# ecker-lab/TreeLearn

Hardware: AMD Instinct MI355X
Metric: Mpoints/sec through sparse U-Net fwd (0.1 m voxel, 40x40 m tile) (higher is better)
Workload: dtype bf16; 1 GPU; config2: single 40x40 m tile, voxel 0.1 m, 1890607 points/tile, 7-level 32-ch sparse U-Net fwd (30.1 M params, random init), 1 tile per GPU; points_per_tile=1890607, tiles_in_flight=4

## Files before the change

### include/treelearn_hip.h

```cpp
#ifndef TREELEARN_HIP_H
#define TREELEARN_HIP_H

#include <stdint.h>

#ifdef __cplusplus
extern "C" {
#endif

typedef void* tl_stream_t;

enum {
  TL_OK = 0,
  TL_ERR_ARG = -1,
  TL_ERR_LAUNCH = -2,
  TL_ERR_UNSUPPORTED = -3
};

enum { TL_F32 = 0, TL_BF16 = 1, TL_F16 = 2 };

int tl_version(void);
int tl_set_tuning(const char* key, int64_t value);
const char* tl_error_string(int code);


// ... 18 lines not shown

int tl_voxel_mean_feats(const float* pf, int C, const int64_t* v2p, int64_t N, int64_t M, int P,
                        int32_t* ws, float* out, tl_stream_t stream);
int tl_voxel_feats(const float* xyz, const float* feats, int F, const int64_t* v2p, int64_t N, int64_t M, int P, int use_coords,
                   int use_feats, int dtype, int32_t* ws, void* out, tl_stream_t stream);


int tl_rulebook_subm(const int32_t* coords, int64_t M, const uint64_t* bitmap, const uint32_t* prefix,
                     const int32_t dims[4], int32_t* nbr, int32_t* compact ,
                     tl_stream_t stream);

int tl_rulebook_down(const int32_t* ccoords, int64_t Mc, const uint64_t* fbitmap, const uint32_t* fprefix,
                     const int32_t fdims[4], int64_t Mf, int32_t* child, int32_t* parent, int32_t* inv, tl_stream_t stream);

int64_t tl_pyramid_ws_words(const int32_t dims0[4], int num_levels, int64_t* level_word_offsets);
int tl_pyramid_build(const int32_t* pcoords, int64_t N, const int32_t dims0[4], const int32_t shape0[3], int num_levels,
                     uint64_t* bitmaps, uint32_t* prefixes, uint32_t* counts, uint32_t* ws, tl_stream_t stream);

typedef struct tl_level {
  int32_t dims[4];
  int64_t n;
  const uint64_t* bitmap;
  const uint32_t* prefix;
  int32_t* coords;
  int32_t* nbr;
  int32_t* compact;
  int32_t* child;
  int32_t* parent;
  int32_t* inv;
  const int32_t* o2n;
  int32_t* inv_packed;
} tl_level;

int tl_rulebooks_build(const tl_level* levels, int num_levels, int32_t* minus_one, int64_t minus_one_words,
                       const int32_t* pcoords, int64_t N, int64_t* v2p, tl_stream_t stream);

#define TL_BLK_HALO_MAX 126
typedef struct tl_blk {
  int32_t* o2n; int32_t* perm; int32_t* coords_new;
  int32_t* unit; int32_t* counter; int32_t* halo; uint32_t* lrb; int32_t* pmask;
  int64_t cap_units;
  int32_t halo_max;
  int32_t reserved;
  int32_t* nn;
} tl_blk;
int64_t tl_blk_ws_words(const int32_t dims[4]);
int tl_blk_build(const uint64_t* bitmap, const uint32_t* prefix, const int32_t dims[4], int64_t n, const tl_blk* out, uint32_t* ws,
                 int phases, tl_stream_t stream);

int tl_rulebook_compact(const int32_t* table, int64_t n, int32_t* compact, tl_stream_t stream);

typedef struct tl_conv_args {
  const void* in;        int64_t in_ld;
  const void* weight;
  const int32_t* table;
  int64_t n_out;         int64_t n_in;
  int32_t K;             int32_t Cin;     int32_t Cout;   int32_t dtype;
  const float* in_scale; const float* in_shift;  int32_t in_relu;  int32_t out_relu;
  const void* residual;  int64_t res_ld;
  const float* out_scale; const float* out_shift;
  void* out;             int64_t out_ld;
  void* out2; int64_t out2_ld; const float* out2_scale; const float* out2_shift; int32_t out2_relu;
  void* out3; int64_t out3_ld; const float* out3_scale; const float* out3_shift; int32_t out3_relu;
  const void* weight_frag;
  int32_t table_one_hot;
  const int32_t* table_compact;
  int32_t in_all_ones;
  int32_t epi_mode;
  double* red_part;
  int32_t* red_nparts;
  const void* bn_x;      int64_t bn_x_ld;
  const float* bn_mean;  const float* bn_rstd;  const float* bn_scale;  const float* bn_shift;  int32_t bn_relu;
  const int32_t* blk_unit; const int32_t* blk_counter; const int32_t* blk_halo; const uint32_t* blk_lrb; const int32_t* blk_pmask;
  const int32_t* table_scatter;
  const void* weight_x3;
} tl_conv_args;

#define TL_EPI_NONE 0
#define TL_EPI_STATS 1
#define TL_EPI_BN_BWD 2
int64_t tl_conv_red_parts(int64_t n_out);

int tl_conv_fwd(const tl_conv_args* args, tl_stream_t stream);

int tl_pack_weight(const float* w_ref, int Cout, int K, int Cin, void* w_packed, int dtype, tl_stream_t stream);
int64_t tl_pack_weight_x3_bytes(int Cout, int K, int Cin);
int tl_pack_weight_x3(const float* w_ref, int Cout, int K, int Cin, void* w_x3, tl_stream_t stream);
int tl_pack_weight_dgrad(const float* w_ref, int Cout, int K, int Cin, int flip, void* w_t, int dtype, tl_stream_t stream);
typedef struct tl_pack_desc {
  const float* src;
  void* dst;
  int32_t Cout, K, Cin, form;
} tl_pack_desc;
int tl_pack_weights_batch(const tl_pack_desc* descs, const int32_t* blocks, int64_t n_blocks, int dtype, tl_stream_t stream);
int tl_pack_weight_frag(const float* w_ref, int Cout, int K, int Cin, void* w_frag, int dtype, tl_stream_t stream);

int64_t tl_conv_wgrad_ws_floats(int64_t n_out, int K, int Cin, int Cout);
int tl_conv_wgrad(const void* x, int64_t x_ld, const void* gout, int64_t g_ld, int dtype, const int32_t* table, int64_t n_out,
                  int64_t n_in, int K, int Cin, int Cout, float* gw, float* ws, tl_stream_t stream);
int tl_conv_wgrad_ref(const void* x, int64_t x_ld, const void* gout, int64_t g_ld, int dtype, const int32_t* table, int64_t n_out,
                      int64_t n_in, int K, int Cin, int Cout, float* gw, float* ws, tl_stream_t stream);

int64_t tl_conv_wgrad_blk_ws_floats(void);
int tl_conv_wgrad_blk(const void* x, int64_t x_ld, const void* gout, int64_t g_ld, int dtype, const int32_t* blk_unit, const int32_t* blk_counter,
                      const int32_t* blk_halo, const uint32_t* blk_lrb, int64_t n, int Cin, int Cout, float* gw, int ref_layout, float* ws,
                      tl_stream_t stream);

int tl_head_mlp(const void* feats, int64_t feats_ld, int dtype, int C, const int64_t* v2p, int64_t N,
                const float* pro_scale, const float* pro_shift,
                const float* w1, const float* b1, const float* w2, const float* b2,
                float* backbone, float* logits, float* offsets, tl_stream_t stream);

int tl_affine_relu(const void* in, int64_t in_ld, void* out, int64_t out_ld, int64_t n, int C, int dtype,
                   const float* scale, const float* shift, int relu, tl_stream_t stream);

int64_t tl_bn_ws_doubles(int64_t n, int C);
int tl_bn_train_stats(const void* x, int64_t ld, int64_t n, int C, int dtype, const float* gamma, const float* beta, float eps,
                      float momentum, double* ws, float* mean, float* rstd, float* scale, float* shift, float* running_mean,
                      float* running_var, int64_t* num_batches_tracked, tl_stream_t stream);
int tl_bn_train_bwd(const void* x, int64_t ld, int x_dtype, const void* dy, int64_t dld, int dy_dtype, int64_t n, int C,
                    const float* mean, const float* rstd, const float* scale, const float* shift, int relu, double* ws,
                    float* dgamma, float* dbeta, void* dx, int64_t xld, const void* dx_add, int64_t dx_add_ld, tl_stream_t stream);

int tl_bn_train_finish(const double* part, int64_t nparts, int64_t n, int C, const float* gamma, const float* beta, float eps, float momentum, float* mean,
                       float* rstd, float* scale, float* shift, float* running_mean, float* running_var, int64_t* num_batches_tracked, tl_stream_t stream);
int tl_bn_train_bwd_from_parts(const void* x, int64_t ld, int x_dtype, const void* g, int64_t gld, int g_dtype, int64_t n, int C, const float* mean,
                               const float* rstd, const float* scale, const float* shift, const double* part, int64_t nparts, float* dgamma, float* dbeta,
                               void* dx, int64_t xld, const void* dx_add, int64_t dx_add_ld, tl_stream_t stream);

int tl_linear_small_f32(const void* x, int64_t x_ld, int dtype, const void* w, int Cin, int Cout, int64_t n, float* out, int64_t out_ld,
                        tl_stream_t stream);

int tl_gather_rows(const void* in, int64_t in_ld, int dtype, int C, int64_t n_rows, const int64_t* idx, int64_t N, void* out, int64_t out_ld, tl_stream_t stream);
int tl_scatter_add_rows(const void* g, int64_t g_ld, int dtype, int C, const int64_t* order, const int64_t* sorted_idx, int64_t N, int64_t n_rows, void* gin,
                        int64_t gin_ld, tl_stream_t stream);

int64_t tl_compact_ws_words(int64_t n);
int tl_compact_rows(const float* in, int C, const uint8_t* mask, int64_t n, float* out, int32_t* count,
                    int32_t* ws, tl_stream_t stream);

typedef struct tl_tile_box {
  float outer[4];
  double inner[4];
  double center[2];
  float half_inner;
} tl_tile_box;
int64_t tl_tile_crop_ws_words(int64_t n);
int tl_tile_crop(const float* xyz, const float* label, const float* feat, int64_t n, int F, const tl_tile_box* box,
                 float* coords, float* out_feat, int64_t* instance_labels, int64_t* semantic_labels,
                 uint8_t* mask_inner, uint8_t* mask_sem, int32_t* count, int32_t* ws, tl_stream_t stream);

int tl_cell_keys(const double* xyz, int64_t n, double cell, double min_bound, const int64_t* base3, int round_input,
                 int64_t* keys, int32_t* err, tl_stream_t stream);
int64_t tl_downsample_ws_words(int64_t n);
int tl_downsample_reduce(const double* xyz, const int64_t* sorted_keys, const int64_t* perm, int64_t n, float* out_xyz,
                         int64_t* first_idx, int64_t* point2vox, int64_t* n_voxels, int32_t* ws, tl_stream_t stream);
int tl_downsample_reduce_r64(const double* xyz, const int64_t* sorted_keys, const int64_t* perm, int64_t n, float* out_xyz,
                             int64_t* first_idx, int64_t* point2vox, int64_t* n_voxels, int32_t* ws, tl_stream_t stream);
int tl_group_mean(const float* src, int64_t n, int C, const int64_t* sorted_keys, const int64_t* perm, double* mean,
                  int64_t* first_idx, int64_t* n_groups, int32_t* ws, tl_stream_t stream);
int tl_verticality(const double* xyz_sorted, const int64_t* sorted_keys, int64_t n, double radius, const int64_t* extent2,
                   float* out, tl_stream_t stream);

int tl_crops_occupancy(const float* xy, int64_t n, const double* x_steps, int x_dim, const double* y_steps, int y_dim, uint8_t* grid,
                       tl_stream_t stream);
int tl_crops_fill(const uint8_t* raw, int x_dim, int y_dim, int how_far_fill, double min_percent_occupied_fill, uint8_t* filled,
// ... 41 lines not shown
                        double* e_w, double* core, void* ws, tl_stream_t stream);
int tl_hdbscan_prim_order_host(const int32_t* e_src, const int32_t* e_dst, const double* e_w, int64_t n, int32_t* o_src,
                               int32_t* o_dst, double* o_w);

int tl_knn_vote(const float* ref_xyz, const int64_t* ref_label, int64_t nr, const float* q_xyz, int64_t nq, int k,
                int64_t* out_label, tl_stream_t stream);
int tl_knn_vote_grid(const float* ref_sorted_xyz, const int64_t* ref_sorted_label, const int64_t* ref_sorted_index, int64_t nr,
                     const int64_t* cell_keys, const int64_t* cell_start, int64_t ncells, const float lo[3], float h, const int32_t dims[3],
                     const float* q_xyz, int64_t nq, int k, int64_t* out_label, tl_stream_t stream);

int tl_eval_contingency(const int64_t* pred, const int64_t* gt, int64_t n, int64_t n_pred, int64_t n_gt, int64_t non_tree_label,
                        int64_t* table, tl_stream_t stream);
enum { TL_EVAL_XY = 0, TL_EVAL_Z = 1 };
int tl_eval_partition(const double* xyz, const int64_t* gt, const int64_t* pred, int64_t n, const int64_t* gt_order, const int64_t* gt_start,
                      int64_t n_gt, const int64_t* pred_order, const int64_t* pred_start, int64_t n_pred, const int64_t* pairs, int64_t m,
                      const double* edges, int n_edges, int mode, int64_t* tp, int64_t* fp, int64_t* fn, double* norm, tl_stream_t stream);

int64_t tl_pointwise_eval_ws_bytes(int64_t n);
int tl_pointwise_eval(const void* logits, const void* offsets, int dtype, const int64_t* semantic_labels, const float* offset_labels,
                      const uint8_t* mask, int64_t n, void* state, void* ws, tl_stream_t stream);

int tl_point_jitter(float* xyz, int64_t n, uint64_t key, tl_stream_t stream);
int64_t tl_train_item_ws_bytes(int64_t n);
int tl_train_item(const float* xyz, const int32_t* instance_label, int64_t n, const double* m, double half_inner, const float* center,
                  int64_t batch_id, int64_t row_offset, float* coords, int64_t* semantic_labels, int64_t* instance_labels,
                  float* offset_labels, uint8_t* masks_inner, uint8_t* masks_off, uint8_t* masks_sem, int64_t* batch_ids, float* centers,
                  void* ws, tl_stream_t stream);

typedef struct {
  double lo[2], h, r, pad, cover_r2, slab_lo, slab_h;
  int32_t nx, ny, nslab, reserved;
} tl_ring_grid;
int tl_ring_lists(const double* ring, int64_t V, const tl_ring_grid* grid, int64_t* cell_cnt, int64_t* slab_cnt, int32_t* cell_seg,
                  int32_t* slab_seg, tl_stream_t stream);
int tl_ring_covered(const double* ring, const tl_ring_grid* grid, const int64_t* cell_start, const int32_t* cell_seg, uint8_t* covered,
                    tl_stream_t stream);
int tl_ring_classify(const void* pts, int dtype_f64, int64_t ld, int64_t n, const double* ring, const tl_ring_grid* grid,
                     const int64_t* slab_start, const int32_t* slab_seg, const int64_t* cell_start, const int32_t* cell_seg,
                     const uint8_t* covered, uint8_t* out, tl_stream_t stream);


#define TL_MAX_LEVELS 8
#define TL_ERR_ARENA (-4)
#define TL_ERR_REACH_ZERO (-5)
#define TL_ERR_BLK (-7)
#define TL_ERR_EXTENT (-6)
typedef struct tl_affine { const float* scale; const float* shift; } tl_affine;
typedef struct tl_weight { const void* w; const void* frag; int32_t K, Cout, Cin, reserved; const void* x3;  } tl_weight;
typedef struct tl_res_desc {
  tl_affine bn0; tl_weight w1; tl_affine bn3; tl_weight w2;
  tl_weight w1x1;
  tl_weight w1_half[2];
} tl_res_desc;
typedef struct tl_ublock_desc {
  int32_t C; int32_t deeper;
  tl_res_desc blocks[2];
  tl_affine bn_down; tl_weight wd;
  tl_affine bn_up; tl_weight wu;
  tl_res_desc tail[2];
  tl_affine bn_cat_l, bn_cat_r;
} tl_ublock_desc;
typedef struct tl_net_desc {
  int32_t dtype;
  int32_t num_levels;
  float voxel_size;
  int32_t has_shape; int32_t spatial_shape[3];
  int32_t blocked;
  int32_t in_channels;
  int32_t use_coords, use_feats;
  int32_t max_points_per_voxel;
  int32_t reserved0;
  tl_weight w_in;
  tl_ublock_desc u[TL_MAX_LEVELS];
  tl_affine out_bn;
  const float* head_w1; const float* head_b1; const float* head_w2; const float* head_b2;
} tl_net_desc;
typedef struct tl_launch_rec {
  int32_t level, kind;
  int32_t K, Cin, Cout, residual, esize, split_part, split_cin, in_prologue;
  int64_t n_out, n_in;
  float ms;
} tl_launch_rec;
typedef struct tl_forward_args {
  const float* xyz; const int64_t* batch_ids; int64_t N; int32_t B; int32_t reserved;
  const float* point_feats;
  void* arena; int64_t arena_bytes;
  float* backbone;
  float* logits; float* offsets;
  tl_stream_t side_stream;
  int64_t needed_bytes;
  int64_t level_n[TL_MAX_LEVELS];
  int32_t blocked_used;
  int32_t launches;
} tl_forward_args;
typedef struct tl_exec tl_exec;
tl_exec* tl_exec_create(void);
void tl_exec_destroy(tl_exec* ex);
int tl_forward(tl_exec* ex, const tl_net_desc* net, tl_forward_args* args, tl_stream_t stream);
int tl_exec_check(tl_exec* ex);
int tl_exec_profile(tl_exec* ex, int enable);
int tl_exec_profile_read(tl_exec* ex, tl_launch_rec* recs, int cap);


#ifdef __cplusplus
}
#endif
#endif
```

### treelearn_amd/_hip.py

```python
import ctypes
import os

import torch

_HERE = os.path.dirname(os.path.abspath(__file__))
LIB_PATH = os.path.join(_HERE, "lib", "libtreelearn_hip.so")

TL_F32, TL_BF16, TL_F16 = 0, 1, 2
TL_OK, TL_ERR_ARG, TL_ERR_UNSUPPORTED = 0, -1, -3
TL_EPI_NONE, TL_EPI_STATS, TL_EPI_BN_BWD = 0, 1, 2
_c = ctypes
_vp, _i64, _i32, _f32 = _c.c_void_p, _c.c_int64, _c.c_int32, _c.c_float


class ConvArgs(_c.Structure):
    _fields_ = [
        ("in_", _vp), ("in_ld", _i64), ("weight", _vp), ("table", _vp),
        ("n_out", _i64), ("n_in", _i64), ("K", _i32), ("Cin", _i32), ("Cout", _i32), ("dtype", _i32),
        ("in_scale", _vp), ("in_shift", _vp), ("in_relu", _i32), ("out_relu", _i32),
        ("residual", _vp), ("res_ld", _i64), ("out_scale", _vp), ("out_shift", _vp),
        ("out", _vp), ("out_ld", _i64),
        ("out2", _vp), ("out2_ld", _i64), ("out2_scale", _vp), ("out2_shift", _vp), ("out2_relu", _i32),
        ("out3", _vp), ("out3_ld", _i64), ("out3_scale", _vp), ("out3_shift", _vp), ("out3_relu", _i32),
        ("weight_frag", _vp), ("table_one_hot", _i32), ("table_compact", _vp),
        ("in_all_ones", _i32), ("epi_mode", _i32), ("red_part", _vp), ("red_nparts", _c.POINTER(_i32)),
        ("bn_x", _vp), ("bn_x_ld", _i64), ("bn_mean", _vp), ("bn_rstd", _vp), ("bn_scale", _vp), ("bn_shift", _vp), ("bn_relu", _i32),
        ("blk_unit", _vp), ("blk_counter", _vp), ("blk_halo", _vp), ("blk_lrb", _vp), ("blk_pmask", _vp), ("table_scatter", _vp),
        ("weight_x3", _vp),
    ]


class TileBox(_c.Structure):
    _fields_ = [("outer", _c.c_float * 4), ("inner", _c.c_double * 4), ("center", _c.c_double * 2), ("half_inner", _c.c_float)]


class Level(_c.Structure):
    _fields_ = [("dims", _c.c_int32 * 4), ("n", _c.c_int64), ("bitmap", _c.c_void_p), ("prefix", _c.c_void_p), ("coords", _c.c_void_p),
                ("nbr", _c.c_void_p), ("compact", _c.c_void_p), ("child", _c.c_void_p), ("parent", _c.c_void_p), ("inv", _c.c_void_p),
                ("o2n", _c.c_void_p), ("inv_packed", _c.c_void_p)]


class Blk(_c.Structure):
    _fields_ = [("o2n", _vp), ("perm", _vp), ("coords_new", _vp), ("unit", _vp), ("counter", _vp), ("halo", _vp), ("lrb", _vp), ("pmask", _vp),
                ("cap_units", _i64), ("halo_max", _i32), ("reserved", _i32), ("nn", _vp)]


class HdbGrid(_c.Structure):
    _fields_ = [("lo", _c.c_double * 2), ("h", _c.c_double), ("levels", _c.c_int32), ("reserved", _c.c_int32)]


TL_MAX_LEVELS = 8
TL_ERR_ARENA, TL_ERR_REACH_ZERO, TL_ERR_EXTENT, TL_ERR_BLK = -4, -5, -6, -7


class Affine(_c.Structure):
    _fields_ = [("scale", _vp), ("shift", _vp)]


class Weight(_c.Structure):
    _fields_ = [("w", _vp), ("frag", _vp), ("K", _i32), ("Cout", _i32), ("Cin", _i32), ("reserved", _i32), ("x3", _vp)]


class ResDesc(_c.Structure):
    _fields_ = [("bn0", Affine), ("w1", Weight), ("bn3", Affine), ("w2", Weight), ("w1x1", Weight), ("w1_half", Weight * 2)]


class UBlockDesc(_c.Structure):
    _fields_ = [("C", _i32), ("deeper", _i32), ("blocks", ResDesc * 2), ("bn_down", Affine), ("wd", Weight), ("bn_up", Affine), ("wu", Weight),
                ("tail", ResDesc * 2), ("bn_cat_l", Affine), ("bn_cat_r", Affine)]


class NetDesc(_c.Structure):
    _fields_ = [("dtype", _i32), ("num_levels", _i32), ("voxel_size", _f32), ("has_shape", _i32), ("spatial_shape", _i32 * 3), ("blocked", _i32),
                ("in_channels", _i32), ("use_coords", _i32), ("use_feats", _i32), ("max_points_per_voxel", _i32), ("reserved0", _i32),
                ("w_in", Weight), ("u", UBlockDesc * TL_MAX_LEVELS), ("out_bn", Affine),
                ("head_w1", _vp), ("head_b1", _vp), ("head_w2", _vp), ("head_b2", _vp)]


class LaunchRec(_c.Structure):
    _fields_ = [("level", _i32), ("kind", _i32), ("K", _i32), ("Cin", _i32), ("Cout", _i32), ("residual", _i32), ("esize", _i32), ("split_part", _i32),
                ("split_cin", _i32), ("in_prologue", _i32), ("n_out", _i64), ("n_in", _i64), ("ms", _f32)]


class ForwardArgs(_c.Structure):
    _fields_ = [("xyz", _vp), ("batch_ids", _vp), ("N", _i64), ("B", _i32), ("reserved", _i32), ("point_feats", _vp), ("arena", _vp), ("arena_bytes", _i64),
                ("backbone", _vp), ("logits", _vp), ("offsets", _vp), ("side_stream", _vp), ("needed_bytes", _i64),
                ("level_n", _i64 * TL_MAX_LEVELS), ("blocked_used", _i32), ("launches", _i32)]


_I4 = _i32 * 4
_I3 = _i32 * 3

PROTOTYPES = {
    "tl_version": (_i32, []),
    "tl_error_string": (_c.c_char_p, [_i32]),
    "tl_set_tuning": (_i32, [_c.c_char_p, _i64]),
    "tl_voxel_point_coords": (_i32, [_vp, _vp, _i64, _i32, _f32, _vp, _vp, _vp, _vp]),
    "tl_voxel_point_coords_one": (_i32, [_vp, _vp, _i64, _f32, _vp, _vp, _vp, _c.POINTER(_i32), _vp]),
    "tl_bitmap_from_points": (_i32, [_vp, _i64, _I4, _vp, _vp]),
    "tl_bitmap_down": (_i32, [_vp, _I4, _I3, _vp, _I4, _vp]),
    "tl_scan_ws_words": (_i64, [_i64]),
    "tl_bitmap_scan": (_i32, [_vp, _i64, _vp, _vp, _vp, _vp]),
    "tl_expand_coords": (_i32, [_vp, _vp, _I4, _vp, _vp]),
    "tl_point_rank": (_i32, [_vp, _i64, _vp, _vp, _I4, _vp, _vp]),
    "tl_voxel_mean_feats": (_i32, [_vp, _i32, _vp, _i64, _i64, _i32, _vp, _vp, _vp]),
    "tl_voxel_feats": (_i32, [_vp, _vp, _i32, _vp, _i64, _i64, _i32, _i32, _i32, _i32, _vp, _vp, _vp]),
    "tl_rulebook_subm": (_i32, [_vp, _i64, _vp, _vp, _I4, _vp, _vp, _vp]),
    "tl_rulebook_down": (_i32, [_vp, _i64, _vp, _vp, _I4, _i64, _vp, _vp, _vp, _vp]),
    "tl_rulebook_compact": (_i32, [_vp, _i64, _vp, _vp]),
    "tl_pyramid_ws_words": (_i64, [_I4, _i32, _c.POINTER(_i64)]),
    "tl_pyramid_build": (_i32, [_vp, _i64, _I4, _I3, _i32, _vp, _vp, _vp, _vp, _vp]),
    "tl_rulebooks_build": (_i32, [_c.POINTER(Level), _i32, _vp, _i64, _vp, _i64, _vp, _vp]),
    "tl_blk_ws_words": (_i64, [_I4]),
    "tl_blk_build": (_i32, [_vp, _vp, _I4, _i64, _c.POINTER(Blk), _vp, _i32, _vp]),
    "tl_conv_fwd": (_i32, [_c.POINTER(ConvArgs), _vp]),
    "tl_conv_red_parts": (_i64, [_i64]),
    "tl_exec_create": (_vp, []),
    "tl_exec_destroy": (None, [_vp]),
    "tl_forward": (_i32, [_vp, _c.POINTER(NetDesc), _c.POINTER(ForwardArgs), _vp]),
    "tl_exec_check": (_i32, [_vp]),
    "tl_exec_profile": (_i32, [_vp, _i32]),
    "tl_exec_profile_read": (_i32, [_vp, _c.POINTER(LaunchRec), _i32]),
    "tl_bn_train_finish": (_i32, [_vp, _i64, _i64, _i32, _vp, _vp, _f32, _f32, _vp, _vp, _vp, _vp, _vp, _vp, _vp, _vp]),
    "tl_bn_train_bwd_from_parts": (_i32, [_vp, _i64, _i32, _vp, _i64, _i32, _i64, _i32, _vp, _vp, _vp, _vp, _vp, _i64, _vp, _vp, _vp, _i64, _vp, _i64, _vp]),
    "tl_pack_weight": (_i32, [_vp, _i32, _i32, _i32, _vp, _i32, _vp]),
    "tl_pack_weight_x3": (_i32, [_vp, _i32, _i32, _i32, _vp, _vp]),
    "tl_pack_weight_x3_bytes": (_i64, [_i32, _i32, _i32]),
    "tl_pack_weight_frag": (_i32, [_vp, _i32, _i32, _i32, _vp, _i32, _vp]),
    "tl_pack_weights_batch": (_i32, [_vp, _vp, _i64, _i32, _vp]),
    "tl_pack_weight_dgrad": (_i32, [_vp, _i32, _i32, _i32, _i32, _vp, _i32, _vp]),
    "tl_conv_wgrad_ws_floats": (_i64, [_i64, _i32, _i32, _i32]),
    "tl_conv_wgrad": (_i32, [_vp, _i64, _vp, _i64, _i32, _vp, _i64, _i64, _i32, _i32, _i32, _vp, _vp, _vp]),
    "tl_conv_wgrad_ref": (_i32, [_vp, _i64, _vp, _i64, _i32, _vp, _i64, _i64, _i32, _i32, _i32, _vp, _vp, _vp]),
    "tl_conv_wgrad_blk_ws_floats": (_i64, []),
    "tl_conv_wgrad_blk": (_i32, [_vp, _i64, _vp, _i64, _i32, _vp, _vp, _vp, _vp, _i64, _i32, _i32, _vp, _i32, _vp, _vp]),
    "tl_head_mlp": (_i32, [_vp, _i64, _i32, _i32, _vp, _i64, _vp, _vp, _vp, _vp, _vp, _vp, _vp, _vp, _vp, _vp]),
    "tl_affine_relu": (_i32, [_vp, _i64, _vp, _i64, _i64, _i32, _i32, _vp, _vp, _i32, _vp]),
    "tl_bn_ws_doubles": (_i64, [_i64, _i32]),
    "tl_bn_train_stats": (_i32, [_vp, _i64, _i64, _i32, _i32, _vp, _vp, _f32, _f32, _vp, _vp, _vp, _vp, _vp, _vp, _vp, _vp, _vp]),
    "tl_bn_train_bwd": (_i32, [_vp, _i64, _i32, _vp, _i64, _i32, _i64, _i32, _vp, _vp, _vp, _vp, _i32, _vp, _vp, _vp, _vp, _i64, _vp, _i64, _vp]),
    "tl_linear_small_f32": (_i32, [_vp, _i64, _i32, _vp, _i32, _i32, _i64, _vp, _i64, _vp]),
    "tl_gather_rows": (_i32, [_vp, _i64, _i32, _i32, _i64, _vp, _i64, _vp, _i64, _vp]),
    "tl_scatter_add_rows": (_i32, [_vp, _i64, _i32, _i32, _vp, _vp, _i64, _i64, _vp, _i64, _vp]),
    "tl_compact_ws_words": (_i64, [_i64]),
    "tl_compact_rows": (_i32, [_vp, _i32, _vp, _i64, _vp, _vp, _vp, _vp]),
    "tl_tile_crop_ws_words": (_i64, [_i64]),
    "tl_tile_crop": (_i32, [_vp, _vp, _vp, _i64, _i32, _vp, _vp, _vp, _vp, _vp, _vp, _vp, _vp, _vp, _vp]),
    "tl_cell_keys": (_i32, [_vp, _i64, _c.c_double, _c.c_double, _vp, _i32, _vp, _vp, _vp]),
    "tl_downsample_ws_words": (_i64, [_i64]),
    "tl_downsample_reduce": (_i32, [_vp, _vp, _vp, _i64, _vp, _vp, _vp, _vp, _vp, _vp]),
    "tl_downsample_reduce_r64": (_i32, [_vp, _vp, _vp, _i64, _vp, _vp, _vp, _vp, _vp, _vp]),
    "tl_group_mean": (_i32, [_vp, _i64, _i32, _vp, _vp, _vp, _vp, _vp, _vp, _vp]),
    "tl_verticality": (_i32, [_vp, _vp, _i64, _c.c_double, _vp, _vp, _vp]),
    "tl_cluster_ws_bytes": (_i64, [_i64]),
    "tl_cluster_grid": (_i32, [_vp, _i64, _c.c_double, _vp, _vp, _vp, _vp]),
    "tl_hdbscan_ws_bytes": (_i64, [_i64]),
    "tl_hdbscan_mst": (_i32, [_vp, _i64, _i32, _vp, _vp, _vp, _vp, _vp, _vp]),
    "tl_hdbscan_labels_host": (_i32, [_vp, _vp, _vp, _i64, _i32, _vp]),
    "tl_hdbscan_prim_order_host": (_i32, [_vp, _vp, _vp, _i64, _vp, _vp, _vp]),
    "tl_hdbscan_grid_plan_ws_bytes": (_i64, []),
    "tl_hdbscan_grid_plan": (_i32, [_vp, _i64, _vp, _vp, _vp]),
    "tl_hdbscan_grid_ws_bytes": (_i64, [_i64, _vp]),
    "tl_hdbscan_grid_ws_bytes_k": (_i64, [_i64, _vp, _i32]),
    "tl_hdbscan_mst_grid": (_i32, [_vp, _i64, _i32, _vp, _vp, _vp, _vp, _vp, _vp, _vp]),
    "tl_knn_vote": (_i32, [_vp, _vp, _i64, _vp, _i64, _i32, _vp, _vp]),
    "tl_knn_vote_grid": (_i32, [_vp, _vp, _vp, _i64, _vp, _vp, _i64, _c.c_float * 3, _f32, _I3, _vp, _i64, _i32, _vp, _vp]),
    "tl_eval_contingency": (_i32, [_vp, _vp, _i64, _i64, _i64, _i64, _vp, _vp]),
    "tl_eval_partition": (_i32, [_vp, _vp, _vp, _i64, _vp, _vp, _i64, _vp, _vp, _i64, _vp, _i64, _vp, _i32, _i32, _vp, _vp, _vp, _vp, _vp]),
    "tl_pointwise_eval_ws_bytes": (_i64, [_i64]),
    "tl_pointwise_eval": (_i32, [_vp, _vp, _i32, _vp, _vp, _vp, _i64, _vp, _vp, _vp]),
    "tl_point_jitter": (_i32, [_vp, _i64, _c.c_uint64, _vp]),
    "tl_train_item_ws_bytes": (_i64, [_i64]),
    "tl_train_item": (_i32, [_vp, _vp, _i64, _c.POINTER(_c.c_double), _c.c_double, _c.POINTER(_f32), _i64, _i64, _vp, _vp, _vp, _vp, _vp, _vp, _vp, _vp, _vp,
                             _vp, _vp]),
    "tl_ring_lists": (_i32, [_vp, _i64, _vp, _vp, _vp, _vp, _vp, _vp]),
    "tl_ring_covered": (_i32, [_vp, _vp, _vp, _vp, _vp, _vp]),
    "tl_crops_occupancy": (_i32, [_vp, _i64, _vp, _i32, _vp, _i32, _vp, _vp]),
    "tl_crops_fill": (_i32, [_vp, _i32, _i32, _i32, _c.c_double, _vp, _vp]),
    "tl_crops_check": (_i32, [_vp, _i32, _vp, _i32, _vp, _vp, _vp, _i64, _c.c_double, _c.c_double, _c.c_double, _vp, _vp, _vp]),
    "tl_crops_ws_words": (_i64, [_i64, _i32]),
    "tl_crops_count": (_i32, [_vp, _i64, _i32, _vp, _vp, _c.c_double, _vp, _vp, _vp]),
    "tl_crops_extract": (_i32, [_vp, _vp, _vp, _i64, _i32, _i32, _vp, _vp, _c.c_double, _vp, _i64, _vp, _vp, _vp, _vp]),
    "tl_outlier_keys": (_i32, [_vp, _i64, _c.c_double * 3, _c.c_double, _I3, _vp, _vp, _vp]),
    "tl_knn_mean_dist": (_i32, [_vp, _vp, _vp, _i64, _c.c_double * 3, _c.c_double, _I3, _i32, _vp, _vp]),
    "tl_sor_ws_doubles": (_i64, [_i64]),
    "tl_sor_keep": (_i32, [_vp, _i64, _c.c_double, _vp, _vp, _vp, _vp]),
    "tl_radius_count": (_i32, [_vp, _vp, _vp, _i64, _c.c_double * 3, _c.c_double, _I3, _c.c_double, _vp, _vp]),
    "tl_ring_classify": (_i32, [_vp, _i32, _i64, _i64, _vp, _vp, _vp, _vp, _vp, _vp, _vp, _vp, _vp]),
}
TL_EVAL_XY, TL_EVAL_Z = 0, 1


class RingGrid(_c.Structure):
    _fields_ = [("lo", _c.c_double * 2), ("h", _c.c_double), ("r", _c.c_double), ("pad", _c.c_double), ("cover_r2", _c.c_double),
                ("slab_lo", _c.c_double), ("slab_h", _c.c_double), ("nx", _i32), ("ny", _i32), ("nslab", _i32), ("reserved", _i32)]

_lib = None

# ... 62 lines not shown
```

### treelearn_amd/csrc/tl_common.h

```cpp
#pragma once
#include <hip/hip_runtime.h>
#include <stdint.h>
#include <atomic>
#include "../../include/treelearn_hip.h"

#define TL_CHECK_LAUNCH()                                   \
  do {                                                      \
    if (hipGetLastError() != hipSuccess) return TL_ERR_LAUNCH; \
  } while (0)

static inline hipStream_t tl_s(tl_stream_t s) { return reinterpret_cast<hipStream_t>(s); }

struct TlAttrOnce {
  std::atomic<uint64_t> done[4];
};
static inline bool tl_lds_attr(TlAttrOnce& once, const void* kernel, int bytes) {
  int dev = 0;
  if (hipGetDevice(&dev) != hipSuccess) return false;
  std::atomic<uint64_t>& w = once.done[(dev >> 6) & 3];
  const uint64_t bit = 1ull << (dev & 63);
  if (w.load(std::memory_order_acquire) & bit) return true;
  if (hipFuncSetAttribute(kernel, hipFuncAttributeMaxDynamicSharedMemorySize, bytes) != hipSuccess) return false;
  w.fetch_or(bit, std::memory_order_release);
  return true;
}

static inline int64_t tl_cdiv(int64_t a, int64_t b) { return (a + b - 1) / b; }

static inline unsigned tl_grid(int64_t work_items, int block) {
  int64_t g = tl_cdiv(work_items, block);
  if (g < 1) g = 1;
  if (g > 256 * 16) g = 256 * 16;
  return (unsigned)g;
}

struct TlDims {
  int B, X, Y, Z, Zw;
};
static inline TlDims tl_dims(const int32_t d[4]) {
  TlDims r{d[0], d[1], d[2], d[3], (d[3] + 63) >> 6};
  return r;
}
__host__ __device__ static inline int64_t tl_nwords(const TlDims& d) { return (int64_t)d.B * d.X * d.Y * d.Zw; }

__device__ __forceinline__ int64_t tl_col_word(const TlDims& d, int b, int x, int y) {
  return (((int64_t)b * d.X + x) * d.Y + y) * d.Zw;
}

__device__ __forceinline__ int tl_rank_at(const uint64_t* __restrict__ bm, const uint32_t* __restrict__ pf,
                                          int64_t wc, int z) {
  const int64_t w = wc + (z >> 6);
  const uint64_t word = bm[w];
  const uint64_t bit = 1ull << (z & 63);
  if (!(word & bit)) return -1;
  return (int)(pf[w] + __popcll(word & (bit - 1)));
}

bool tl_conv_one_hot_direct_enabled(int64_t n_out);
```

### treelearn_amd/csrc/tl_conv.hip

```cpp
#include "tl_conv_internal.h"
#include <atomic>
#include <string.h>

namespace {

template <typename T>
__global__ void __launch_bounds__(256) k_conv_generic(ConvP p) {
  const T* in = (const T*)p.in; const T* w = (const T*)p.w; const T* res = (const T*)p.res;
  const int64_t total = p.n_out * p.Cout;
  for (int64_t t = (int64_t)blockIdx.x * blockDim.x + threadIdx.x; t < total; t += (int64_t)gridDim.x * blockDim.x) {
    const int64_t o = t / p.Cout; const int j = (int)(t % p.Cout);
    float acc = 0.f;
    for (int k = 0; k < p.K; ++k) {
      const int64_t idx = p.table ? (int64_t)p.table[(int64_t)k * p.n_out + o] : o;
      if (idx < 0) continue;
      const T* x = in + idx * p.in_ld;
      const T* wr = w + ((int64_t)k * p.Cout + j) * p.Cin;
      for (int c = 0; c < p.Cin; ++c) {
        float v = ld_elem(x + c);
        if (p.in_scale) v = fmaf(v, p.in_scale[c], p.in_shift[c]);
        if (p.in_relu) v = fmaxf(v, 0.f);
        if (sizeof(T) == 2) v = __bfloat162float(__float2bfloat16(v));
        acc = fmaf(v, ld_elem(wr + c), acc);
      }
// ... 237 lines not shown
    else reinterpret_cast<__hip_bfloat16*>(d.dst)[t] = __float2bfloat16(v);
  }
}

template <typename T>
__global__ void k_affine_relu(const T* __restrict__ in, int64_t in_ld, T* __restrict__ out, int64_t out_ld, int64_t n, int C,
                              const float* __restrict__ scale, const float* __restrict__ shift, int relu) {
  const int64_t total = n * C;
  for (int64_t t = (int64_t)blockIdx.x * blockDim.x + threadIdx.x; t < total; t += (int64_t)gridDim.x * blockDim.x) {
    const int64_t r = t / C; const int c = (int)(t % C);
    float v = ld_elem(in + r * in_ld + c);
    if (scale) v = fmaf(v, scale[c], shift[c]);
    if (relu) v = fmaxf(v, 0.f);
    st_elem(out + r * out_ld + c, v);
  }
}

template <int T16>
__global__ void __launch_bounds__(256) k_affine_relu_v8(const void* __restrict__ in, int64_t in_ld, void* __restrict__ out, int64_t out_ld, int64_t n, int C,
                                                        const float* __restrict__ scale, const float* __restrict__ shift, int relu) {
  const int vpr = C >> 3;
  const int64_t total = n * vpr, stride = (int64_t)gridDim.x * 256;
  int64_t v = (int64_t)blockIdx.x * 256 + threadIdx.x;
  if (v >= total) return;
  const int c0 = (int)(v % vpr) * 8;
  float sc[8], sh[8];
#pragma unroll
  for (int q = 0; q < 8; ++q) { sc[q] = scale ? scale[c0 + q] : 1.f; sh[q] = scale ? shift[c0 + q] : 0.f; }
  for (; v < total; v += stride) {
    const int64_t r = v / vpr;
    float x[8];
    typedef _Float16 hx2 __attribute__((ext_vector_type(2)));
    if constexpr (T16 == 1) {
      const u32x4 q4 = __builtin_nontemporal_load(reinterpret_cast<const u32x4*>((const uint16_t*)in + r * in_ld + c0));
#pragma unroll
      for (int q = 0; q < 4; ++q) { x[2 * q] = bf16_lo(q4[q]); x[2 * q + 1] = bf16_hi(q4[q]); }
    } else if constexpr (T16 == 2) {
      const u32x4 q4 = *reinterpret_cast<const u32x4*>((const uint16_t*)in + r * in_ld + c0);
      const uint32_t w0 = q4[0], w1 = q4[1], w2 = q4[2], w3 = q4[3];
      const uint32_t ws[4] = {w0, w1, w2, w3};
#pragma unroll
      for (int q = 0; q < 4; ++q) { const hx2 h = __builtin_bit_cast(hx2, ws[q]); x[2 * q] = (float)h[0]; x[2 * q + 1] = (float)h[1]; }
    } else {
      const f32x4* s4 = reinterpret_cast<const f32x4*>((const float*)in + r * in_ld + c0);
      const f32x4 a = __builtin_nontemporal_load(s4), b = __builtin_nontemporal_load(s4 + 1);
#pragma unroll
      for (int q = 0; q < 4; ++q) { x[q] = a[q]; x[q + 4] = b[q]; }
    }
#pragma unroll
    for (int q = 0; q < 8; ++q) { x[q] = fmaf(x[q], sc[q], sh[q]); if (relu) x[q] = fmaxf(x[q], 0.f); }
    if constexpr (T16 == 1) {
      u32x4 o;
#pragma unroll
      for (int q = 0; q < 4; ++q) o[q] = pack_bf16x2(x[2 * q], x[2 * q + 1]);
      *reinterpret_cast<u32x4*>((uint16_t*)out + r * out_ld + c0) = o;
    } else if constexpr (T16 == 2) {
      u32x4 o;
#pragma unroll
      for (int q = 0; q < 4; ++q) { const hx2 h = {(_Float16)x[2 * q], (_Float16)x[2 * q + 1]}; o[q] = __builtin_bit_cast(uint32_t, h); }
      *reinterpret_cast<u32x4*>((uint16_t*)out + r * out_ld + c0) = o;
    } else {
      f32x4* d = reinterpret_cast<f32x4*>((float*)out + r * out_ld + c0);
      d[0] = f32x4{x[0], x[1], x[2], x[3]}; d[1] = f32x4{x[4], x[5], x[6], x[7]};
    }
  }
}

}

static int64_t g_small_rows = kSmallRows;
extern int g_small_mode;
extern int g_wgrad_dense;
extern int64_t g_wgrad_dense_min_rows;
extern int g_wgrad_rows;
extern int g_wgrad_dma;
static int g_stream = 1;
static int g_streamq = 1;
static int g_streamq_x3 = 1;
static int g_direct = 1;
static int g_direct_oh = 1;
static int g_blk = 1;
static int g_up = 1;

bool tl_conv_one_hot_direct_enabled(int64_t n_out) { return g_direct && g_direct_oh && n_out > g_small_rows; }

extern "C" {

int tl_set_tuning(const char* key, int64_t value) {
  if (!key) return TL_ERR_ARG;
  if (!strcmp(key, "direct")) { g_direct = (int)value; return TL_OK; }
  if (!strcmp(key, "blk")) { g_blk = (int)value; return TL_OK; }
  if (!strcmp(key, "up")) { g_up = (int)value; return TL_OK; }
  if (!strcmp(key, "direct_oh")) { g_direct_oh = (int)value; return TL_OK; }
  if (!strcmp(key, "stream")) { g_stream = (int)value; return TL_OK; }
  if (!strcmp(key, "streamq")) { g_streamq = (int)value; return TL_OK; }
  if (!strcmp(key, "streamq_x3")) { if (value != 0 && value != 1) return TL_ERR_ARG; g_streamq_x3 = (int)value; return TL_OK; }
  if (!strcmp(key, "small_rows")) { g_small_rows = value; return TL_OK; }
  if (!strcmp(key, "small_mode")) { g_small_mode = (int)value; return TL_OK; }
  if (!strcmp(key, "wgrad_dense")) { g_wgrad_dense = (int)value; return TL_OK; }
  if (!strcmp(key, "wgrad_rows")) { g_wgrad_rows = (int)value; return TL_OK; }
  if (!strcmp(key, "wgrad_dma")) { g_wgrad_dma = (int)value; return TL_OK; }
  if (!strcmp(key, "wgrad_dense_min_rows")) { g_wgrad_dense_min_rows = value; return TL_OK; }
  return TL_ERR_ARG;
}

int tl_conv_fwd(const tl_conv_args* a, tl_stream_t stream) {
  if (!a || !a->in || !a->weight || !a->out || a->n_out <= 0 || a->K <= 0 || a->K > 27 || a->Cin <= 0 || a->Cout <= 0) return TL_ERR_ARG;
  const bool has_blk = a->blk_unit && a->blk_counter && a->blk_halo && a->blk_lrb && a->K == 27;
  if (!a->table && a->K != 1 && !has_blk && !(a->in_all_ones && a->blk_pmask)) return TL_ERR_ARG;
  if ((a->in_scale == nullptr) != (a->in_shift == nullptr)) return TL_ERR_ARG;
  if ((a->out_scale == nullptr) != (a->out_shift == nullptr)) return TL_ERR_ARG;
  if (a->dtype != TL_F32 && a->dtype != TL_BF16 && a->dtype != TL_F16) return TL_ERR_ARG;
  const bool f16 = a->dtype == TL_F16;
  const int dt = f16 ? TL_BF16 : a->dtype;
  const auto L_direct = f16 ? tl_launch_conv_direct_f16 : tl_launch_conv_direct;
  const auto L_ones27 = f16 ? tl_launch_conv_ones27_f16 : tl_launch_conv_ones27;
  const auto L_stream = f16 ? tl_launch_conv_stream_f16 : tl_launch_conv_stream;
  const auto L_streamq = f16 ? tl_launch_conv_streamq_f16 : tl_launch_conv_streamq;
  const auto L_small = f16 ? tl_launch_conv_small_f16 : tl_launch_conv_small;
  const auto L_tinycin = f16 ? tl_launch_conv_tinycin_f16 : tl_launch_conv_tinycin;
  const auto L_blk = f16 ? tl_launch_conv_blk_f16 : tl_launch_conv_blk;
  const auto L_up = f16 ? tl_launch_conv_up_f16 : tl_launch_conv_up;
  ConvP p;
  p.in = a->in; p.in_ld = a->in_ld; p.w = a->weight; p.w_frag = a->weight_frag;
  p.w_x3 = (a->dtype == TL_F32 && a->Cin % 32 == 0 && ((uintptr_t)a->weight_x3) % 16 == 0) ? a->weight_x3 : nullptr; p.table = a->table; p.ctab = (a->K == 27) ? a->table_compact : nullptr; p.n_out = a->n_out; p.n_in = a->n_in;
  p.K = a->K; p.Cin = a->Cin; p.Cout = a->Cout; p.in_scale = a->in_scale; p.in_shift = a->in_shift;
  p.in_relu = a->in_relu; p.out_relu = a->out_relu; p.res = a->residual; p.res_ld = a->res_ld;
  p.out_scale = a->out_scale; p.out_shift = a->out_shift; p.out = a->out; p.out_ld = a->out_ld;
  p.out2 = a->out2; p.out2_ld = a->out2_ld; p.out2_scale = a->out2_scale; p.out2_shift = a->out2_shift; p.out2_relu = a->out2_relu;
  p.out3 = a->out3; p.out3_ld = a->out3_ld; p.out3_scale = a->out3_scale; p.out3_shift = a->out3_shift; p.out3_relu = a->out3_relu;
  if ((a->out2_scale == nullptr) != (a->out2_shift == nullptr) || (a->out3_scale == nullptr) != (a->out3_shift == nullptr)) return TL_ERR_ARG;
  p.nblk = (int)tl_cdiv(a->n_out, TM);
  p.one_hot = a->table != nullptr ? a->table_one_hot : 0;
  p.blk_unit = has_blk ? a->blk_unit : nullptr; p.blk_counter = a->blk_counter; p.blk_halo = a->blk_halo; p.blk_lrb = a->blk_lrb;
  p.blk_pmask = a->K == 27 ? a->blk_pmask : nullptr;
  p.epi_mode = a->epi_mode; p.red_part = a->red_part; p.red_nparts = a->red_nparts; p.bn_x = a->bn_x; p.bn_x_ld = a->bn_x_ld;
  p.bn_mean = a->bn_mean; p.bn_rstd = a->bn_rstd; p.bn_scale = a->bn_scale; p.bn_shift = a->bn_shift; p.bn_relu = a->bn_relu;
  const bool train = a->epi_mode != TL_EPI_NONE;
  if (train) {
    if ((a->epi_mode != TL_EPI_STATS && a->epi_mode != TL_EPI_BN_BWD) || !a->red_part || ((uintptr_t)a->red_part) % 8) return TL_ERR_ARG;
    if (a->epi_mode == TL_EPI_BN_BWD) {
      if (!a->bn_x || !a->bn_mean || !a->bn_rstd || !a->bn_scale || !a->bn_shift) return TL_ERR_ARG;
      if (a->bn_x_ld % 8 || ((uintptr_t)a->bn_x) % 16 || ((uintptr_t)a->bn_mean) % 16 || ((uintptr_t)a->bn_rstd) % 16 || ((uintptr_t)a->bn_scale) % 16 ||
          ((uintptr_t)a->bn_shift) % 16)
        return TL_ERR_UNSUPPORTED;
    }
    if (a->red_nparts) *a->red_nparts = 0;
  }
  hipStream_t s = tl_s(stream);
  if (p.one_hot == 2) {
    const bool shape = a->K == 8 && a->Cin == 64 && a->Cout == 32 && !train && !a->in_scale && !a->in_relu && g_direct && g_direct_oh;
    if (!shape || !(dt == TL_BF16 || (dt == TL_F32 && p.w_x3))) return TL_ERR_UNSUPPORTED;
    return L_direct(p, dt, s);
  }
  const bool vec_ok = (a->in_ld % 8 == 0) && (((uintptr_t)a->in) % 16 == 0) && (((uintptr_t)a->weight) % 16 == 0);
  const bool out_vec = (a->out_ld % 8 == 0) && (((uintptr_t)a->out) % 16 == 0) &&
                       (!a->out2 || (a->out2_ld % 8 == 0 && ((uintptr_t)a->out2) % 16 == 0)) && (!a->out3 || (a->out3_ld % 8 == 0 && ((uintptr_t)a->out3) % 16 == 0));
  if (a->in_all_ones && !train && (dt == TL_BF16 || (dt == TL_F32 && !f16)) && out_vec && (g_direct || !a->table) && ((uintptr_t)a->weight) % 4 == 0 && !a->residual) {
    const int rc = L_ones27(p, dt, s);
    if (rc != TL_ERR_UNSUPPORTED) return rc;
  }
  if (has_blk && dt == TL_BF16 && g_blk && vec_ok && out_vec && (!a->residual || (a->res_ld % 8 == 0 && ((uintptr_t)a->residual) % 16 == 0)) &&
      (!a->out_scale || (((uintptr_t)a->out_scale) % 4 == 0 && ((uintptr_t)a->out_shift) % 4 == 0)) && (!a->in_relu || a->in_scale)) {
    const int rc = L_blk(p, s);
    if (rc != TL_ERR_UNSUPPORTED) return rc;
  }
  if (has_blk && a->dtype == TL_F32 && p.w_x3 && g_blk && !train) {
    const int rc = tl_launch_conv_blk_x3(p, s);
    if (rc != TL_ERR_UNSUPPORTED) return rc;
  }
  if (!a->table && a->K != 1) return TL_ERR_UNSUPPORTED;
  if (a->table_scatter && p.one_hot && g_up && !train && dt == TL_BF16 && vec_ok && out_vec &&
      (!a->out_scale || (((uintptr_t)a->out_scale) % 16 == 0 && ((uintptr_t)a->out_shift) % 16 == 0))) {
    const int rc = L_up(p, a->table_scatter, s);
    if (rc != TL_ERR_UNSUPPORTED) return rc;
  }
  if (dt == TL_BF16 && a->Cin == 4 && a->Cout == 32 && g_direct && out_vec && ((uintptr_t)a->in) % 8 == 0 && ((uintptr_t)a->weight) % 16 == 0 &&
      (!a->residual || (a->res_ld % 8 == 0 && ((uintptr_t)a->residual) % 16 == 0))) {
    const int rc = L_direct(p, TL_BF16, s);
    if (rc != TL_ERR_UNSUPPORTED) return rc;
  }
  if (!train && a->Cin <= 8 && a->Cout % 8 == 0 && a->Cout <= 64 && !a->in_scale && !a->in_relu && out_vec) return L_tinycin(p, dt, s);
  if (!train && vec_ok && a->n_out <= g_small_rows && a->Cin % 32 == 0 && a->Cout % 32 == 0) return L_small(p, dt, s);
  if (train && a->n_out <= g_small_rows) return TL_ERR_UNSUPPORTED;
  const bool aligned = (a->in_ld % 4 == 0) && (((uintptr_t)a->in) % 16 == 0) && (((uintptr_t)a->weight) % 16 == 0) &&
                       (!a->in_scale || (((uintptr_t)a->in_scale) % 16 == 0 && ((uintptr_t)a->in_shift) % 16 == 0));
  if (p.w_x3 && a->Cin >= 256) {
    if (dt == TL_F32 && !train && g_stream && aligned && out_vec && a->Cin % 64 == 0 && a->Cout % 32 == 0 && !a->in_scale && !a->in_relu && !a->residual &&
        !a->out2 && !a->out3 && a->n_out > g_small_rows && (!a->out_scale || (((uintptr_t)a->out_scale) % 16 == 0 && ((uintptr_t)a->out_shift) % 16 == 0))) {
      ConvP p1 = p;
      p1.Cin = a->Cin / 2; p1.out_scale = nullptr; p1.out_shift = nullptr; p1.out_relu = 0;
      const int rc1 = L_stream(p1, TL_F32, s);
      if (rc1 == TL_OK) {
        ConvP p2 = p;
        p2.Cin = a->Cin / 2; p2.in = static_cast<const float*>(a->in) + a->Cin / 2;
        p2.w_x3 = static_cast<const char*>(p.w_x3) + (size_t)a->K * a->Cout * (a->Cin / 2) * 4;
        p2.res = a->out; p2.res_ld = a->out_ld;
        return L_stream(p2, TL_F32, s);
      }
      if (rc1 != TL_ERR_UNSUPPORTED) return rc1;
    }
    p.w_x3 = nullptr;
  }
  if (dt == TL_F32 && aligned && out_vec && a->Cin % 32 == 0 && a->Cout % 32 == 0 && !a->in_scale && !a->in_relu &&
      (!a->residual || (a->res_ld % 4 == 0 && ((uintptr_t)a->residual) % 16 == 0)) &&
      (!a->out_scale || (((uintptr_t)a->out_scale) % 16 == 0 && ((uintptr_t)a->out_shift) % 16 == 0))) {
    if (g_direct) { const int rc = L_direct(p, TL_F32, s); if (rc != TL_ERR_UNSUPPORTED) return rc; }
    if (g_stream && g_streamq && g_streamq_x3 && p.w_x3 && !train && a->n_out > g_small_rows) {
      const int rc = tl_launch_conv_streamq_x3(p, s);
      if (rc != TL_ERR_UNSUPPORTED) return rc;
    }
    if (g_stream) { const int rc = L_stream(p, TL_F32, s); if (rc != TL_ERR_UNSUPPORTED) return rc; }
  }
  if (train && dt == TL_F32) return TL_ERR_UNSUPPORTED;
  if (dt == TL_F32 && !f16 && vec_ok && a->n_out <= 4 * g_small_rows && a->Cin % 32 == 0 && a->Cout % 32 == 0 && !a->in_scale && !a->in_relu)
    return L_small(p, dt, s);
  if (dt == TL_F32 && aligned && a->Cin % KC == 0 && a->Cout % 32 == 0 && a->Cout <= 224) {
    switch (a->Cout / 32) {
      case 1: return launch_mfma_f32<1>(p, s);
      case 2: return launch_mfma_f32<2>(p, s);
      case 3: return launch_mfma_f32<3>(p, s);
      case 4: return launch_mfma_f32<4>(p, s);
      case 5: return launch_mfma_f32<5>(p, s);
      case 6: return launch_mfma_f32<6>(p, s);
      case 7: return launch_mfma_f32<7>(p, s);
    }
  }
  if (dt == TL_BF16 && aligned && vec_ok && out_vec && a->Cin % 32 == 0 && a->Cout % 32 == 0 && a->Cout <= 224 &&
      (!a->residual || (a->res_ld % 8 == 0 && ((uintptr_t)a->residual) % 16 == 0)) &&
      (!a->out_scale || (((uintptr_t)a->out_scale) % 16 == 0 && ((uintptr_t)a->out_shift) % 16 == 0)))
  {
    if (p.one_hot && g_direct && g_direct_oh && a->K == 8 && a->Cin == 64 && a->Cout == 32) {
      const int rc = L_direct(p, TL_BF16, s);
      if (rc != TL_ERR_UNSUPPORTED) return rc;
    }
    if (p.one_hot && g_stream && a->K == 8) {
      const int rc = L_stream(p, TL_BF16, s);
      if (rc != TL_ERR_UNSUPPORTED) return rc;
    }
    if (g_direct) {
      const int rc = L_direct(p, TL_BF16, s);
      if (rc != TL_ERR_UNSUPPORTED) return rc;
    }
    if (g_stream && g_streamq) {
      const int rc = L_streamq(p, s);
      if (rc != TL_ERR_UNSUPPORTED) return rc;
    }
    if (g_stream) {
      const int rc = L_stream(p, TL_BF16, s);
      if (rc != TL_ERR_UNSUPPORTED) return rc;
    }
    if (train) return TL_ERR_UNSUPPORTED;
    return f16 ? tl_launch_conv_bf16_f16(p, s) : tl_launch_conv_bf16(p, s);
  }
  if (train || f16) return TL_ERR_UNSUPPORTED;
  {
    const int rc = tl_launch_conv_tinycout(p, dt, s);
    if (rc != TL_ERR_UNSUPPORTED) return rc;
  }
  const unsigned g = tl_grid(a->n_out * a->Cout, 256);
  if (dt == TL_F32) k_conv_generic<float><<<g, 256, 0, s>>>(p);
  else k_conv_generic<__hip_bfloat16><<<g, 256, 0, s>>>(p);
  TL_CHECK_LAUNCH();
  return TL_OK;
}

int64_t tl_conv_red_parts(int64_t n_out) {
  const int64_t a = tl_cdiv(n_out > 0 ? n_out : 1, 256);
  return a > 2048 ? a : 2048;
}

int tl_pack_weight(const float* w_ref, int Cout, int K, int Cin, void* w_packed, int dtype, tl_stream_t stream) {
  if (!w_ref || !w_packed || Cout <= 0 || K <= 0 || Cin <= 0 || (dtype != TL_F32 && dtype != TL_BF16 && dtype != TL_F16)) return TL_ERR_ARG;
  k_pack_weight<<<tl_grid((int64_t)Cout * K * Cin, 256), 256, 0, tl_s(stream)>>>(w_ref, Cout, K, Cin, w_packed, dtype);
  TL_CHECK_LAUNCH();
  return TL_OK;
}

int64_t tl_pack_weight_x3_bytes(int Cout, int K, int Cin) {
  if (Cout <= 0 || K <= 0 || Cin <= 0 || Cin % 32) return -1;
  const int64_t one = (int64_t)K * Cout * Cin * 4;
  return (Cin < 256 && Cout % 32 == 0) ? 2 * one : one;
}

int tl_pack_weight_x3(const float* w_ref, int Cout, int K, int Cin, void* w_x3, tl_stream_t stream) {
  if (!w_ref || !w_x3 || Cout <= 0 || K <= 0 || Cin <= 0 || Cin % 32) return TL_ERR_ARG;
  k_pack_weight_x3<<<tl_grid((int64_t)Cout * K * Cin * 2, 256), 256, 0, tl_s(stream)>>>(w_ref, Cout, K, Cin, reinterpret_cast<uint16_t*>(w_x3));
  TL_CHECK_LAUNCH();
  return TL_OK;
}

int tl_pack_weight_dgrad(const float* w_ref, int Cout, int K, int Cin, int flip, void* w_t, int dtype, tl_stream_t stream) {
  if (!w_ref || !w_t || Cout <= 0 || K <= 0 || Cin <= 0 || (dtype != TL_F32 && dtype != TL_BF16 && dtype != TL_F16)) return TL_ERR_ARG;
  k_pack_weight_dgrad<<<tl_grid((int64_t)Cout * K * Cin, 256), 256, 0, tl_s(stream)>>>(w_ref, Cout, K, Cin, flip, w_t, dtype);
  TL_CHECK_LAUNCH();
  return TL_OK;
}

int tl_pack_weights_batch(const tl_pack_desc* descs, const int32_t* blocks, int64_t n_blocks, int dtype, tl_stream_t stream) {
  if (!descs || !blocks || n_blocks <= 0 || n_blocks > 0x7FFFFFFF || (dtype != TL_F32 && dtype != TL_BF16 && dtype != TL_F16)) return TL_ERR_ARG;
  k_pack_batch<<<(unsigned)n_blocks, 256, 0, tl_s(stream)>>>(descs, reinterpret_cast<const int2*>(blocks), dtype);
  TL_CHECK_LAUNCH();
  return TL_OK;
}

int tl_pack_weight_frag(const float* w_ref, int Cout, int K, int Cin, void* w_frag, int dtype, tl_stream_t stream) {
  if (!w_ref || !w_frag || Cout <= 0 || K <= 0 || Cin <= 0 || Cout % 32 || Cin % 32 || (dtype != TL_F32 && dtype != TL_BF16 && dtype != TL_F16)) return TL_ERR_ARG;
  k_pack_weight_frag<<<tl_grid((int64_t)Cout * K * Cin / 8, 256), 256, 0, tl_s(stream)>>>(w_ref, Cout, K, Cin, w_frag, dtype);
  TL_CHECK_LAUNCH();
  return TL_OK;
}

int tl_affine_relu(const void* in, int64_t in_ld, void* out, int64_t out_ld, int64_t n, int C, int dtype, const float* scale,
                   const float* shift, int relu, tl_stream_t stream) {
  if (!in || !out || n <= 0 || C <= 0 || (scale == nullptr) != (shift == nullptr)) return TL_ERR_ARG;
  if ((dtype == TL_F32 || dtype == TL_BF16 || dtype == TL_F16) && C % 8 == 0 && in_ld % 8 == 0 && out_ld % 8 == 0 && ((uintptr_t)in) % 16 == 0 && ((uintptr_t)out) % 16 == 0) {
    const int vpr = C / 8;
    int64_t gv = tl_cdiv(n * vpr, 256 * 4);
    if (gv > 256 * 16) gv = 256 * 16;
    gv = tl_cdiv(gv * 256, (int64_t)vpr * 256) * vpr;
    if (dtype == TL_BF16) k_affine_relu_v8<1><<<(unsigned)gv, 256, 0, tl_s(stream)>>>(in, in_ld, out, out_ld, n, C, scale, shift, relu);
    else if (dtype == TL_F16) k_affine_relu_v8<2><<<(unsigned)gv, 256, 0, tl_s(stream)>>>(in, in_ld, out, out_ld, n, C, scale, shift, relu);
    else k_affine_relu_v8<0><<<(unsigned)gv, 256, 0, tl_s(stream)>>>(in, in_ld, out, out_ld, n, C, scale, shift, relu);
    TL_CHECK_LAUNCH();
    return TL_OK;
  }
  const unsigned g = tl_grid(n * C, 256);
  if (dtype == TL_F32) k_affine_relu<float><<<g, 256, 0, tl_s(stream)>>>((const float*)in, in_ld, (float*)out, out_ld, n, C, scale, shift, relu);
  else if (dtype == TL_BF16) k_affine_relu<__hip_bfloat16><<<g, 256, 0, tl_s(stream)>>>((const __hip_bfloat16*)in, in_ld, (__hip_bfloat16*)out, out_ld, n, C, scale, shift, relu);
  else if (dtype == TL_F16) k_affine_relu<_Float16><<<g, 256, 0, tl_s(stream)>>>((const _Float16*)in, in_ld, (_Float16*)out, out_ld, n, C, scale, shift, relu);
  else return TL_ERR_ARG;
  TL_CHECK_LAUNCH();
  return TL_OK;
}

}
```

### treelearn_amd/csrc/tl_conv_direct.hip

```cpp
#include "tl_conv_internal.h"
#include <atomic>

namespace {


template <bool BF16, int K, int NB, int UN, int G, int WAVES, bool CT = false, bool TR = false, bool OH = false, bool X3 = false>
__global__ void __launch_bounds__(WAVES * 64) k_conv_direct(ConvP p, int ntiles, int walk) {
  static_assert(!X3 || (!BF16 && !TR), "the split-bf16 contraction: fp32 rows, inference");
  constexpr int EB = BF16 ? 2 : 4;
  constexpr int UB = 32 * EB;
  constexpr int NJ = UB / 32;
  constexpr int SLOTS = UB / 16;
  constexpr int COUT = NB * 32;
  constexpr int NG = (K + G - 1) / G;
  constexpr int EP = COUT + 4;
  extern __shared__ __attribute__((aligned(16))) char smem[];
  char* Ws = smem;
  float* Es = reinterpret_cast<float*>(smem + (size_t)K * UN * COUT * UB);
  double* Ds = reinterpret_cast<double*>(smem + (size_t)K * UN * COUT * UB + (size_t)WAVES * 32 * EP * 4);

  const int tid = threadIdx.x, lane = tid & 63, wv = tid >> 6;
  const int fi = lane & 31, fh = lane >> 5;
  auto swz_of = [](int n) { return BF16 ? ((n >> 2) & 3) : ((n >> 1) & 7); };

// ... 332 lines not shown
      acc = h16_mfma(af, bfrag[s], acc);
    }
#pragma unroll
    for (int r = 0; r < 16; ++r) ew[((r & 3) + 8 * (r >> 2) + 4 * fh) * EP + fi] = acc[r];
    __builtin_amdgcn_fence(__ATOMIC_RELEASE, "wavefront");
    __builtin_amdgcn_wave_barrier();
    if constexpr (TR) {
      float r0 = 0.f, r1 = 0.f;
      epi_block32<true, EP>(p, ew, lane, (int64_t)tile * 32, 0, r0, r1);
      if (lane < 32) { Ds[wv][0][lane] += (double)r0; Ds[wv][1][lane] += (double)r1; }
    } else {
#pragma unroll
      for (int e0 = 0; e0 < 2; ++e0) {
        const int e = lane + e0 * 64, rr = e >> 2, cvv = e & 3;
        const int64_t orow = (int64_t)tile * 32 + rr;
        if (orow < p.n_out) {
          const f32x4 v0 = *reinterpret_cast<const f32x4*>(ew + rr * EP + cvv * 8), v1 = *reinterpret_cast<const f32x4*>(ew + rr * EP + cvv * 8 + 4);
          float v[8] = {v0[0], v0[1], v0[2], v0[3], v1[0], v1[1], v1[2], v1[3]};
          epi_views8<true>(p, orow, cvv * 8, v);
        }
      }
    }
    __builtin_amdgcn_fence(__ATOMIC_RELEASE, "wavefront");
    __builtin_amdgcn_wave_barrier();
  }
  if constexpr (TR) {
    __syncthreads();
    for (int e = threadIdx.x; e < 64; e += WAVES * 64) {
      double t = 0.0;
      for (int w = 0; w < WAVES; ++w) t += Ds[w][e >> 5][e & 31];
      p.red_part[(int64_t)blockIdx.x * 64 + e] = t;
    }
  }
}

template <bool BF16>
__global__ void __launch_bounds__(256) k_conv_ones27(ConvP p) {
  __shared__ __attribute__((aligned(16))) float S[27][32];
  for (int e = threadIdx.x; e < 27 * 32; e += 256) {
    float t = 0.f;
    if constexpr (BF16) {
      const uint16_t* w = (const uint16_t*)p.w;
      for (int c = 0; c < p.Cin; ++c) t += bf16_lo((uint32_t)w[(int64_t)e * p.Cin + c]);
    } else {
      const float* w = (const float*)p.w;
      for (int c = 0; c < p.Cin; ++c) t += w[(int64_t)e * p.Cin + c];
    }
    S[e >> 5][e & 31] = t;
  }
  __syncthreads();
  const int32_t* mask = p.blk_pmask ? p.blk_pmask : p.ctab + (int64_t)9 * p.n_out;
  const int64_t total = p.n_out * 4;
  for (int64_t t = (int64_t)blockIdx.x * 256 + threadIdx.x; t < total; t += (int64_t)gridDim.x * 256) {
    const int64_t row = t >> 2; const int c0 = (int)(t & 3) * 8;
    uint32_t m = (uint32_t)mask[row];
    float v[8] = {0.f, 0.f, 0.f, 0.f, 0.f, 0.f, 0.f, 0.f};
    while (m) {
      const int k = __builtin_ctz(m); m &= m - 1;
      const f32x4 a = *reinterpret_cast<const f32x4*>(&S[k][c0]), b = *reinterpret_cast<const f32x4*>(&S[k][c0 + 4]);
#pragma unroll
      for (int q = 0; q < 4; ++q) { v[q] += a[q]; v[q + 4] += b[q]; }
    }
    epi_views8<BF16>(p, row, c0, v);
  }
}

template <bool BF16, int K, int NB, int UN, int G, int WAVES, bool CT = false, bool TR = false, bool OH = false, bool X3 = false>
int launch(const ConvP& p_, hipStream_t s) {
  ConvP p = p_;
  if constexpr (X3) {
    if (p.epi_mode != TL_EPI_NONE) return TL_ERR_UNSUPPORTED;
    p.w = p.w_x3;
  }
  if constexpr (!TR && BF16) {
    if (p.epi_mode != TL_EPI_NONE) return launch<BF16, K, NB, UN, G, WAVES, CT, true, OH>(p, s);
  } else if constexpr (!TR) {
    if (p.epi_mode != TL_EPI_NONE) return TL_ERR_UNSUPPORTED;
  }
  if constexpr (TR && NB >= 3) return TL_ERR_UNSUPPORTED;
  else {
  constexpr int UB = BF16 ? 64 : 128;
  const size_t lds = (size_t)K * UN * NB * 32 * UB + (size_t)WAVES * 32 * (NB * 32 + 4) * 4 + (TR ? (size_t)WAVES * 2 * NB * 32 * 8 : 0);
  if (lds > 160 * 1024) return TL_ERR_UNSUPPORTED;
  static TlAttrOnce attr_once;
  if (!tl_lds_attr(attr_once, reinterpret_cast<const void*>(&k_conv_direct<BF16, K, NB, UN, G, WAVES, CT, TR, OH, X3>), 160 * 1024)) return TL_ERR_LAUNCH;
  const int ntiles = (int)tl_cdiv(p.n_out, 32);
  const int per_cu = (int)((160 * 1024) / lds) < 1 ? 1 : (int)((160 * 1024) / lds);
  int grid = 256 * (per_cu > 2 ? 2 : per_cu);
  const int need = (int)tl_cdiv(ntiles, WAVES);
  if (grid > need) grid = need;
  k_conv_direct<BF16, K, NB, UN, G, WAVES, CT, TR, OH, X3><<<grid, WAVES * 64, lds, s>>>(p, ntiles, 0);
  if (p.red_nparts) *p.red_nparts = grid;
  return hipGetLastError() == hipSuccess ? TL_OK : TL_ERR_LAUNCH;
  }
}

template <bool BF16, int K, int G>
int dispatch(const ConvP& p, hipStream_t s) {
  const int nb = p.Cout / 32, un = p.Cin / 32;
  const size_t wbytes = (size_t)K * p.Cout * p.Cin * (BF16 ? 2 : 4);
  if constexpr (BF16 && K == 27) {
    if (p.ctab && nb == 1 && un == 1) return launch<true, 27, 1, 1, G, 16, true>(p, s);
    if (p.ctab && nb == 1 && un == 2) return launch<true, 27, 1, 2, G, 8, true>(p, s);
  }
  if constexpr (BF16 && K == 8) {
    if (p.one_hot && nb == 1 && un == 2) return launch<true, 8, 1, 2, G, 16, false, false, true>(p, s);
  }
  if constexpr (BF16 && K == 1) {
    if (nb == 2 && un == 4) return launch<true, 1, 2, 4, 1, 16>(p, s);
    if (nb == 3 && un == 6) return launch<true, 1, 3, 6, 1, 8>(p, s);
    if (nb == 4 && un == 8) return launch<true, 1, 4, 8, 1, 8>(p, s);
  }
  if constexpr (!BF16 && K == 1) {
    if (nb == 2 && un == 4 && p.epi_mode == TL_EPI_NONE) {
      if (p.w_x3) return launch<false, 1, 2, 4, 1, 8, false, false, false, true>(p, s);
      return launch<false, 1, 2, 4, 1, 8>(p, s);
    }
  }
  if constexpr (!BF16 && K == 8) {
    if (p.one_hot && p.w_x3 && p.epi_mode == TL_EPI_NONE && nb == 1 && un == 2) return launch<false, 8, 1, 2, G, 12, false, false, true, true>(p, s);
  }
#define TL_D(NB_, UN_)                                                                                               \
  if (nb == NB_ && un == UN_) {                                                                                      \
    if constexpr (BF16) return wbytes <= 64 * 1024 ? launch<true, K, NB_, UN_, G, 16>(p, s) : launch<true, K, NB_, UN_, G, 8>(p, s); \
    else {                                                                                                           \
      if (p.w_x3 && p.epi_mode == TL_EPI_NONE)        \
        return launch<false, K, NB_, UN_, (G > 2 ? 2 : G), (K == 27 && NB_ == 1 && UN_ == 1 ? 11 : 8), false, false, false, true>(p, s);         \
      return launch<false, K, NB_, UN_, (G > 2 ? 2 : G), 8>(p, s);                                                   \
    }                                                                                                                \
  }
  TL_D(1, 1) TL_D(1, 2) TL_D(2, 1) TL_D(2, 2) TL_D(2, 3) TL_D(3, 2) TL_D(1, 3) TL_D(3, 1)
#undef TL_D
  return TL_ERR_UNSUPPORTED;
}

}

int tl_launch_conv_ones27(const ConvP& p, int dtype, hipStream_t s) {
  if (p.K != 27 || p.Cout != 32 || (!p.ctab && !p.blk_pmask) || p.Cin <= 0 || p.Cin > 64 || p.in_scale || p.in_relu || p.epi_mode != TL_EPI_NONE) return TL_ERR_UNSUPPORTED;
  if (dtype == TL_BF16) k_conv_ones27<true><<<tl_grid(p.n_out * 4, 256), 256, 0, s>>>(p);
  else k_conv_ones27<false><<<tl_grid(p.n_out * 4, 256), 256, 0, s>>>(p);
  return hipGetLastError() == hipSuccess ? TL_OK : TL_ERR_LAUNCH;
}


int tl_launch_conv_direct(const ConvP& p, int dtype, hipStream_t s) {
  if (p.in_scale || p.in_relu) return TL_ERR_UNSUPPORTED;
  if (p.one_hot == 2 && !(p.K == 8 && p.Cin == 64 && p.Cout == 32 && p.epi_mode == TL_EPI_NONE && (dtype == TL_BF16 || p.w_x3))) return TL_ERR_UNSUPPORTED;
  const int eb = dtype == TL_BF16 ? 2 : 4;
  if (dtype == TL_BF16 && p.Cin == 4 && p.Cout == 32 && p.K <= 28 && p.table && p.in_ld % 4 == 0 && (int64_t)p.n_in * p.in_ld * 2 < 0xFFFF0000ll) {
    const int ntiles = (int)tl_cdiv(p.n_out, 32);
    int grid = (int)tl_cdiv(ntiles, 8);
    if (grid > 2048) grid = 2048;
    if (p.epi_mode != TL_EPI_NONE) {
      if (p.ctab && p.K == 27) k_conv_in4<8, true, true><<<grid, 512, 0, s>>>(p, ntiles);
      else k_conv_in4<8, false, true><<<grid, 512, 0, s>>>(p, ntiles);
    } else if (p.ctab && p.K == 27) k_conv_in4<8, true><<<grid, 512, 0, s>>>(p, ntiles);
    else k_conv_in4<8><<<grid, 512, 0, s>>>(p, ntiles);
    if (p.red_nparts) *p.red_nparts = grid;
    return hipGetLastError() == hipSuccess ? TL_OK : TL_ERR_LAUNCH;
  }
  if (p.Cin % 32 || p.Cout % 32) return TL_ERR_UNSUPPORTED;
  const int64_t ld_b = p.in_ld * eb, in_bytes = (p.n_in - 1) * ld_b + (int64_t)p.Cin * eb;
  if (!(in_bytes > 0 && in_bytes + 2 * ld_b < 0xFFFFFFFFll)) return TL_ERR_UNSUPPORTED;
  if ((size_t)p.K * p.Cout * p.Cin * eb > 112 * 1024) return TL_ERR_UNSUPPORTED;
  if (dtype == TL_BF16) {
    switch (p.K) {
      case 27: return dispatch<true, 27, 3>(p, s);
      case 8: return dispatch<true, 8, 2>(p, s);
      case 1: return dispatch<true, 1, 1>(p, s);
    }
  } else {
    switch (p.K) {
      case 27: return dispatch<false, 27, 3>(p, s);
      case 8: return dispatch<false, 8, 2>(p, s);
      case 1: return dispatch<false, 1, 1>(p, s);
    }
  }
  return TL_ERR_UNSUPPORTED;
}
```

### treelearn_amd/csrc/tl_conv_internal.h

```cpp
#pragma once
#include "tl_common.h"
#include <hip/hip_bf16.h>
#include "tl_half.h"

#ifdef TL_F16_BUILD
#define tl_launch_conv_direct tl_launch_conv_direct_f16
#define tl_launch_conv_ones27 tl_launch_conv_ones27_f16
#define tl_launch_conv_stream tl_launch_conv_stream_f16
#define tl_launch_conv_streamq tl_launch_conv_streamq_f16
#define tl_launch_conv_small tl_launch_conv_small_f16
#define tl_launch_conv_tinycin tl_launch_conv_tinycin_f16
#define tl_launch_conv_bf16 tl_launch_conv_bf16_f16
#define tl_launch_conv_blk tl_launch_conv_blk_f16
#define tl_launch_conv_up tl_launch_conv_up_f16
#define g_small_mode g_small_mode_f16
#endif

typedef float f32x16 __attribute__((ext_vector_type(16)));
typedef float f32x4 __attribute__((ext_vector_type(4)));
typedef uint32_t u32x4 __attribute__((ext_vector_type(4)));
typedef short s16x8 __attribute__((ext_vector_type(8)));

struct ConvP {
  const void* in; int64_t in_ld;
  const void* w;
  const void* w_frag;
  const void* w_x3;
  const int32_t* table;
  const int32_t* ctab;
  int64_t n_out, n_in;
  int K, Cin, Cout;
  const float* in_scale; const float* in_shift; int in_relu, out_relu;
  const void* res; int64_t res_ld;
  const float* out_scale; const float* out_shift;
  void* out; int64_t out_ld;
  void* out2; int64_t out2_ld; const float* out2_scale; const float* out2_shift; int out2_relu;
  void* out3; int64_t out3_ld; const float* out3_scale; const float* out3_shift; int out3_relu;
  int nblk;
  int epi_mode;
  double* red_part;
  int32_t* red_nparts;
  const void* bn_x; int64_t bn_x_ld;
  const float* bn_mean; const float* bn_rstd; const float* bn_scale; const float* bn_shift; int bn_relu;
  int one_hot;
  const int32_t* blk_unit; const int32_t* blk_counter; const int32_t* blk_halo; const uint32_t* blk_lrb; const int32_t* blk_pmask;
};

static __device__ __forceinline__ float ld_elem(const float* p) { return *p; }
static __device__ __forceinline__ float ld_elem(const __hip_bfloat16* p) { return h16_lo((uint32_t)*reinterpret_cast<const uint16_t*>(p)); }
static __device__ __forceinline__ void st_elem(float* p, float v) { *p = v; }
static __device__ __forceinline__ float ld_elem(const _Float16* p) { return (float)*p; }
static __device__ __forceinline__ void st_elem(_Float16* p, float v) { *p = (_Float16)v; }
static __device__ __forceinline__ void st_elem(__hip_bfloat16* p, float v) { *reinterpret_cast<uint16_t*>(p) = (uint16_t)(h16_pack2(v, 0.f) & 0xFFFFu); }

static __device__ __forceinline__ int xcd_tile(int b, int n) {
  const int q = n >> 3, r = n & 7, x = b & 7, i = b >> 3;
  return (x < r ? x * (q + 1) : r * (q + 1) + (x - r) * q) + i;
}


typedef __bf16 bf16x8 __attribute__((ext_vector_type(8)));

static __device__ __forceinline__ uint32_t pack_bf16x2(float lo, float hi) { return h16_pack2(lo, hi); }
static __device__ __forceinline__ float bf16_lo(uint32_t u) { return h16_lo(u); }
static __device__ __forceinline__ float bf16_hi(uint32_t u) { return h16_hi(u); }

template <bool BF16>
static __device__ __forceinline__ void epi_store1(void* base, int64_t ld, const float* sc, const float* sh, int relu, int64_t row, int j, float y) {
  if (sc) y = fmaf(y, sc[j], sh[j]);
  if (relu) y = fmaxf(y, 0.f);
  if constexpr (BF16) ((uint16_t*)base)[row * ld + j] = (uint16_t)(pack_bf16x2(y, 0.f) & 0xFFFFu);
  else ((float*)base)[row * ld + j] = y;
}
template <bool BF16>
static __device__ __forceinline__ void epi_store8(void* base, int64_t ld, const float* sc, const float* sh, int relu, int64_t row, int c0, const float (&y)[8]) {
  float v[8];
#pragma unroll
  for (int q = 0; q < 8; ++q) v[q] = y[q];
  if (sc) {
    const f32x4 a0 = *reinterpret_cast<const f32x4*>(sc + c0), a1 = *reinterpret_cast<const f32x4*>(sc + c0 + 4);
    const f32x4 b0 = *reinterpret_cast<const f32x4*>(sh + c0), b1 = *reinterpret_cast<const f32x4*>(sh + c0 + 4);
#pragma unroll
    for (int q = 0; q < 4; ++q) { v[q] = fmaf(v[q], a0[q], b0[q]); v[q + 4] = fmaf(v[q + 4], a1[q], b1[q]); }
  }
  if (relu) {
#pragma unroll
    for (int q = 0; q < 8; ++q) v[q] = fmaxf(v[q], 0.f);
  }
  if constexpr (BF16) {
    u32x4 o;
#pragma unroll
    for (int q = 0; q < 4; ++q) o[q] = pack_bf16x2(v[2 * q], v[2 * q + 1]);
    *reinterpret_cast<u32x4*>((uint16_t*)base + row * ld + c0) = o;
  } else {
    f32x4* d = reinterpret_cast<f32x4*>((float*)base + row * ld + c0);
    d[0] = f32x4{v[0], v[1], v[2], v[3]}; d[1] = f32x4{v[4], v[5], v[6], v[7]};
  }
}

template <bool BF16>
static __device__ __forceinline__ void mma16(f32x16& acc, const u32x4& a, const u32x4& b) {
  if constexpr (BF16) {
    acc = h16_mfma(a, b, acc);
  } else {
    const f32x4 af = __builtin_bit_cast(f32x4, a), bf = __builtin_bit_cast(f32x4, b);
    acc = __builtin_amdgcn_mfma_f32_32x32x2f32(af[0], bf[0], acc, 0, 0, 0);
    acc = __builtin_amdgcn_mfma_f32_32x32x2f32(af[1], bf[1], acc, 0, 0, 0);
    acc = __builtin_amdgcn_mfma_f32_32x32x2f32(af[2], bf[2], acc, 0, 0, 0);
    acc = __builtin_amdgcn_mfma_f32_32x32x2f32(af[3], bf[3], acc, 0, 0, 0);
  }
}
static __device__ __forceinline__ uint32_t x3_pack2(float a, float b) {
  typedef __bf16 v2 __attribute__((ext_vector_type(2)));
  const v2 v = {(__bf16)a, (__bf16)b};
  return __builtin_bit_cast(uint32_t, v);
}
static __device__ __forceinline__ void x3_split8(const u32x4& a0, const u32x4& a1, u32x4& hi, u32x4& lo) {
#pragma unroll
  for (int q = 0; q < 2; ++q) {
    const uint32_t u0 = a0[2 * q], u1 = a0[2 * q + 1], v0 = a1[2 * q], v1 = a1[2 * q + 1];
    hi[q] = __builtin_amdgcn_perm(u1, u0, 0x07060302u);
    hi[2 + q] = __builtin_amdgcn_perm(v1, v0, 0x07060302u);
    lo[q] = x3_pack2(__uint_as_float(u0) - __uint_as_float(u0 & 0xFFFF0000u), __uint_as_float(u1) - __uint_as_float(u1 & 0xFFFF0000u));
    lo[2 + q] = x3_pack2(__uint_as_float(v0) - __uint_as_float(v0 & 0xFFFF0000u), __uint_as_float(v1) - __uint_as_float(v1 & 0xFFFF0000u));
  }
}
static __device__ __forceinline__ void mma16_x3(f32x16& acc, const u32x4& ah, const u32x4& al, const u32x4& bh, const u32x4& bl) {
  acc = __builtin_amdgcn_mfma_f32_32x32x16_bf16(__builtin_bit_cast(bf16x8, al), __builtin_bit_cast(bf16x8, bh), acc, 0, 0, 0);
  acc = __builtin_amdgcn_mfma_f32_32x32x16_bf16(__builtin_bit_cast(bf16x8, ah), __builtin_bit_cast(bf16x8, bl), acc, 0, 0, 0);
// ... 198 lines not shown
```

### treelearn_amd/csrc/tl_conv_stream.hip

```cpp
#include "tl_conv_internal.h"
#include <atomic>

namespace {

constexpr int WAVES = 8;
constexpr int NT = WAVES * 64;

template <bool BF16, int K, int NB, int UN, int DA, int RB, int OCC, bool OH = false, bool X3 = false>
__global__ void __launch_bounds__(NT, OCC) k_conv_stream(ConvP p) {
  static_assert(!X3 || !BF16, "the split-bf16 contraction reads fp32 rows");
  constexpr int EB = BF16 ? 2 : 4, UB = 32 * EB, NJ = UB / 32, SLOTS = UB / 16;
  constexpr int COUT = NB * 32, CIN = UN * 32;
  constexpr int BROW = CIN * EB + 16;
  constexpr int BSLOTS = UN * SLOTS;
  constexpr int BVEC = COUT * BSLOTS;
  constexpr int BPT = (BVEC + NT - 1) / NT;
  constexpr int EP = 32 + 4;
  constexpr int WROWS = 32 * RB;
  extern __shared__ __attribute__((aligned(16))) char smem[];
  char* Bs = smem;
  float* Es = reinterpret_cast<float*>(smem);

  const int tid = threadIdx.x, lane = tid & 63, wv = tid >> 6;
  const int fi = lane & 31, fh = lane >> 5;
// ... 97 lines not shown
#pragma unroll
        for (int J = 0; J < 2; ++J) {
          u32x4 ah[RB], al[RB];
          if constexpr (OH) {
#pragma unroll
            for (int rb = 0; rb < RB; ++rb) {
              if (k == 0) x3_split8(a1[rb][c][2 * J], a1[rb][c][2 * J + 1], ah1[rb][c][J], al1[rb][c][J]);
              const bool mine = idx[k][rb] >= 0;
#pragma unroll
              for (int q = 0; q < 4; ++q) { ah[rb][q] = mine ? ah1[rb][c][J][q] : 0u; al[rb][q] = mine ? al1[rb][c][J][q] : 0u; }
            }
          } else {
#pragma unroll
            for (int rb = 0; rb < RB; ++rb) x3_split8(a[k % DA][rb][c][2 * J], a[k % DA][rb][c][2 * J + 1], ah[rb], al[rb]);
          }
          u32x4 bh[NB], blo[NB];
#pragma unroll
          for (int nb = 0; nb < NB; ++nb) {
            const char* bp = bl + nb * 32 * BROW + (c * SLOTS + 2 * J + fh) * 16;
            bh[nb] = *reinterpret_cast<const u32x4*>(bp); blo[nb] = *reinterpret_cast<const u32x4*>(bp + 64);
          }
#pragma unroll
          for (int rb = 0; rb < RB; ++rb) {
#pragma unroll
            for (int nb = 0; nb < NB; ++nb) acc[rb][nb] = __builtin_amdgcn_mfma_f32_32x32x16_bf16(__builtin_bit_cast(bf16x8, al[rb]), __builtin_bit_cast(bf16x8, bh[nb]), acc[rb][nb], 0, 0, 0);
#pragma unroll
            for (int nb = 0; nb < NB; ++nb) acc[rb][nb] = __builtin_amdgcn_mfma_f32_32x32x16_bf16(__builtin_bit_cast(bf16x8, ah[rb]), __builtin_bit_cast(bf16x8, blo[nb]), acc[rb][nb], 0, 0, 0);
#pragma unroll
            for (int nb = 0; nb < NB; ++nb) acc[rb][nb] = __builtin_amdgcn_mfma_f32_32x32x16_bf16(__builtin_bit_cast(bf16x8, ah[rb]), __builtin_bit_cast(bf16x8, bh[nb]), acc[rb][nb], 0, 0, 0);
          }
        }
    } else
#pragma unroll
    for (int c = 0; c < UN; ++c)
#pragma unroll
      for (int j = 0; j < NJ; ++j) {
#pragma unroll
        for (int nb = 0; nb < NB; ++nb) {
          const int slot = c * SLOTS + 2 * j + fh;
          const u32x4 bf = *reinterpret_cast<const u32x4*>(bl + nb * 32 * BROW + slot * 16);
#pragma unroll
          for (int rb = 0; rb < RB; ++rb) {
            if constexpr (OH) {
              const u32x4 z = {0u, 0u, 0u, 0u};
              mma16<BF16>(acc[rb][nb], idx[k][rb] >= 0 ? a1[rb][c][j] : z, bf);
            } else mma16<BF16>(acc[rb][nb], a[k % DA][rb][c][j], bf);
          }
        }
      }
    if constexpr (!OH) { if (k + DA < K) issue_a(k + DA, a[k % DA]); }
    if (k + 1 < K) __syncthreads();
  }

  __syncthreads();
  float* ew = Es + wv * 32 * EP;
  float red0[NB], red1[NB];
#pragma unroll
  for (int nb = 0; nb < NB; ++nb) { red0[nb] = 0.f; red1[nb] = 0.f; }
#pragma unroll
  for (int rb = 0; rb < RB; ++rb)
#pragma unroll
    for (int nb = 0; nb < NB; ++nb) {
#pragma unroll
      for (int r = 0; r < 16; ++r) ew[((r & 3) + 8 * (r >> 2) + 4 * fh) * EP + fi] = acc[rb][nb][r];
      __builtin_amdgcn_fence(__ATOMIC_RELEASE, "wavefront");
      __builtin_amdgcn_wave_barrier();
      epi_block32<BF16, EP>(p, ew, lane, r0 + rb * 32, nb * 32, red0[nb], red1[nb]);
      __builtin_amdgcn_fence(__ATOMIC_RELEASE, "wavefront");
      __builtin_amdgcn_wave_barrier();
    }
  if (p.epi_mode != TL_EPI_NONE) epi_finish_wg<WAVES, EP, NB>(p, Es, tid, red0, red1);
}

template <bool BF16, int K, int NB, int UN, int DA, int RB, bool OH = false, bool X3 = false>
int launch(ConvP p, hipStream_t s) {
  if constexpr (X3) p.w = p.w_x3;
  constexpr int EB = BF16 ? 2 : 4;
  constexpr int BPTL = (NB * 32 * UN * (BF16 ? 4 : 8) + NT - 1) / NT;
  constexpr int VG = RB * NB * 16 + DA * RB * UN * (BF16 ? 8 : 16) + (K <= 8 ? 8 : 27) * RB + 4 * BPTL * (DA > 2 ? DA - 1 : 1) + 20;
  constexpr int OCC = (OH && X3) ? 2 : ((VG <= 120 || (X3 && NB * UN <= 4)) ? 4 : 2);
  const size_t wt = 2 * (size_t)NB * 32 * (UN * 32 * EB + 16), ep = (size_t)WAVES * 32 * 36 * 4;
  const size_t lds = wt > ep ? wt : ep;
  if (lds > 160 * 1024) return TL_ERR_UNSUPPORTED;
  static TlAttrOnce attr_once;
  if (!tl_lds_attr(attr_once, reinterpret_cast<const void*>(&k_conv_stream<BF16, K, NB, UN, DA, RB, OCC, OH, X3>), 160 * 1024)) return TL_ERR_LAUNCH;
  p.nblk = (int)tl_cdiv(p.n_out, WAVES * 32 * RB);
  k_conv_stream<BF16, K, NB, UN, DA, RB, OCC, OH, X3><<<p.nblk, NT, lds, s>>>(p);
  if (p.red_nparts) *p.red_nparts = p.nblk;
  return hipGetLastError() == hipSuccess ? TL_OK : TL_ERR_LAUNCH;
}

template <bool BF16, int K>
int dispatch(const ConvP& p, hipStream_t s) {
  const int nb = p.Cout / 32, un = p.Cin / 32;
  if constexpr (BF16 && K == 8) {
    if (p.one_hot) {
      if (nb == 2 && un == 3) return launch<true, 8, 2, 3, 1, 1, true>(p, s);
      if (nb == 1 && un == 2) return launch<true, 8, 1, 2, 1, 1, true>(p, s);
      if (nb == 3 && un == 4) return launch<true, 8, 3, 4, 1, 1, true>(p, s);
    }
  }
  if constexpr (!BF16 && K == 8) {
    if (p.one_hot == 1 && p.w_x3 && p.epi_mode == TL_EPI_NONE) {
      if (nb == 2 && un == 3) return launch<false, 8, 2, 3, 1, 1, true, true>(p, s);
      if (nb == 3 && un == 4) return launch<false, 8, 3, 4, 1, 1, true, true>(p, s);
    }
  }
  if constexpr (BF16 && K == 8) {
    if (!p.one_hot && nb == 2 && un == 1) return launch<true, 8, 2, 1, 3, 2>(p, s);
  }
#define TL_S(NB_, UN_, DB_, RB_, DF_)                                                                \
  if (nb == NB_ && un == UN_) {                                                                      \
    if constexpr (BF16) return launch<true, K, NB_, UN_, DB_, RB_>(p, s);                            \
    else {                                                                                           \
      if (p.w_x3) return launch<false, K, NB_, UN_, 1, 1, false, true>(p, s);    \
      return launch<false, K, NB_, UN_, DF_, 1>(p, s);                                               \
    }                                                                                                \
  }
  TL_S(2, 2, 3, 1, 2) TL_S(2, 4, 2, 1, 1) TL_S(3, 3, 1, 2, 1) TL_S(3, 6, 1, 1, 1) TL_S(4, 4, 2, 1, 1) TL_S(2, 3, 3, 1, 1) TL_S(3, 2, 3, 1, 2)
  TL_S(3, 4, 2, 1, 1) TL_S(4, 3, 2, 1, 1) TL_S(1, 2, 3, 1, 2) TL_S(2, 1, 3, 1, 2) TL_S(1, 1, 3, 1, 2)
#undef TL_S
  return TL_ERR_UNSUPPORTED;
}

}

int tl_launch_conv_stream(const ConvP& p, int dtype, hipStream_t s) {
  if (p.in_scale || p.in_relu) return TL_ERR_UNSUPPORTED;
  const int eb = dtype == TL_BF16 ? 2 : 4;
  const int64_t ld_b = p.in_ld * eb, in_bytes = (p.n_in - 1) * ld_b + (int64_t)p.Cin * eb;
  if (!(in_bytes > 0 && in_bytes + 2 * ld_b < 0xFFFFFFFFll)) return TL_ERR_UNSUPPORTED;
  if (dtype == TL_BF16) {
    switch (p.K) {
      case 27: return dispatch<true, 27>(p, s);
      case 8: return dispatch<true, 8>(p, s);
    }
  } else {
    switch (p.K) {
      case 27: return dispatch<false, 27>(p, s);
      case 8: return dispatch<false, 8>(p, s);
    }
  }
  return TL_ERR_UNSUPPORTED;
}
```

### treelearn_amd/csrc/tl_conv_streamq.hip

```cpp
#include "tl_conv_internal.h"
#include <atomic>
#include <type_traits>

namespace {

template <int CTRL>
static __device__ __forceinline__ uint32_t qperm(uint32_t v) {
  return (uint32_t)__builtin_amdgcn_mov_dpp((int)v, CTRL, 0xf, 0xf, true);
}

static __device__ __forceinline__ void quad_transpose(const u32x4 (&S)[4], u32x4 (&F)[4], bool o0, bool o1) {
  u32x4 T[4];
#pragma unroll
  for (int i1 = 0; i1 < 2; ++i1)
#pragma unroll
    for (int d = 0; d < 4; ++d) {
      const uint32_t P = S[2 * i1][d], Q = S[2 * i1 + 1][d];
      const uint32_t Pn = qperm<0xB1>(P), Qn = qperm<0xB1>(Q);
      T[2 * i1][d] = o0 ? Qn : P;
      T[2 * i1 + 1][d] = o0 ? Q : Pn;
    }
#pragma unroll
  for (int x0 = 0; x0 < 2; ++x0)
#pragma unroll
// ... 152 lines not shown
    for (int pp = 0; pp < PN; ++pp)
#pragma unroll
      for (int s = 0; s < 4; ++s)
#pragma unroll
        for (int nb = 0; nb < NB; ++nb) {
          const u32x4 bf = *reinterpret_cast<const u32x4*>(bl + nb * 32 * BROW + (pp * 8 + s) * 16);
#pragma unroll
          for (int rb = 0; rb < RB; ++rb) {
            mma16<true>(acc[rb][nb], F[rb][pp][s], bf);
          }
        }
    if (k + DA < KV) { issue_a(k + DA, a[U % DA]); if (k + DA + 1 < KV) read_idx(k + DA + 1); }
    if (k + 1 < KV) __syncthreads();
  };
  if constexpr (X3 && !UL) {
    for (int k0 = 0; k0 < KV; k0 += 2) {
      step(k0, std::integral_constant<int, 0>{});
      if (k0 + 1 < KV) step(k0 + 1, std::integral_constant<int, 1>{});
    }
  } else if constexpr (X3) {
#pragma unroll
    for (int k = 0; k < KV; ++k) {
      if ((k & 1) == 0) step(k, std::integral_constant<int, 0>{});
      else step(k, std::integral_constant<int, 1>{});
    }
  } else {
#pragma unroll
  for (int k = 0; k < KV; ++k) {
    if (k + 1 < KV) store_b((k + 1) & 1, bw[(k + 1) % RW]);
    if (k + WA < KV) load_b(k + WA, bw[(k + WA) % RW]);
    __builtin_amdgcn_sched_barrier(0);
    u32x4 F[RB][PN][4];
#pragma unroll
    for (int rb = 0; rb < RB; ++rb)
#pragma unroll
      for (int pp = 0; pp < PN; ++pp) {
        quad_transpose(a[k % DA][rb][pp], F[rb][pp], o0, o1);
      }
    const char* bl = Bs + (k & 1) * COUT * BROW + fi * BROW + fh * 64;
#pragma unroll
    for (int pp = 0; pp < PN; ++pp)
#pragma unroll
      for (int s = 0; s < 4; ++s)
#pragma unroll
        for (int nb = 0; nb < NB; ++nb) {
          const u32x4 bf = *reinterpret_cast<const u32x4*>(bl + nb * 32 * BROW + (pp * 8 + s) * 16);
#pragma unroll
          for (int rb = 0; rb < RB; ++rb) {
            mma16<true>(acc[rb][nb], F[rb][pp][s], bf);
          }
        }
    if (k + DA < KV) { issue_a(k + DA, a[k % DA]); if (k + DA + 1 < KV) read_idx(k + DA + 1); }
    if (k + 1 < KV) __syncthreads();
  }
  }

  __syncthreads();
  float* ew = Es + wv * 32 * EP;
  float red0[NB], red1[NB];
#pragma unroll
  for (int nb = 0; nb < NB; ++nb) { red0[nb] = 0.f; red1[nb] = 0.f; }
#pragma unroll
  for (int rb = 0; rb < RB; ++rb)
#pragma unroll
    for (int nb = 0; nb < NB; ++nb) {
#pragma unroll
      for (int r = 0; r < 16; ++r) ew[(2 * (r >> 2) + fh + 8 * (r & 3)) * EP + fi] = acc[rb][nb][r];
      __builtin_amdgcn_fence(__ATOMIC_RELEASE, "wavefront");
      __builtin_amdgcn_wave_barrier();
      epi_block32<!X3, EP>(p, ew, lane, r0 + rb * 32, nb * 32, red0[nb], red1[nb]);
      __builtin_amdgcn_fence(__ATOMIC_RELEASE, "wavefront");
      __builtin_amdgcn_wave_barrier();
    }
  if (p.epi_mode != TL_EPI_NONE) epi_finish_wg<W, EP, NB>(p, Es, tid, red0, red1);
}

template <int K, int NB, int PN, int DA, int W = 8, int RB = 1, int SP = 1, bool X3 = false, bool UL = false>
int launch(ConvP p, hipStream_t s) {
  constexpr int OCC = 2;
  if constexpr (X3) p.w = p.w_x3;
  const size_t wt = 2 * (size_t)NB * 32 * (PN * 128 + 16) + (size_t)W * K * 32 * RB * 4, ep = (size_t)W * 32 * 36 * 4;
  const size_t lds = wt > ep ? wt : ep;
  if (lds > 160 * 1024) return TL_ERR_UNSUPPORTED;
  static TlAttrOnce attr_once;
  if (!tl_lds_attr(attr_once, reinterpret_cast<const void*>(&k_conv_streamq<K, NB, PN, DA, W, RB, OCC, SP, X3, UL>), 160 * 1024)) return TL_ERR_LAUNCH;
  p.nblk = (int)tl_cdiv(p.n_out, W * 32 * RB);
  k_conv_streamq<K, NB, PN, DA, W, RB, OCC, SP, X3, UL><<<p.nblk, W * 64, lds, s>>>(p);
  if (p.red_nparts) *p.red_nparts = p.nblk;
  return hipGetLastError() == hipSuccess ? TL_OK : TL_ERR_LAUNCH;
}

}

int tl_launch_conv_streamq(const ConvP& p, hipStream_t s) {
  if (p.in_scale || p.in_relu || p.Cin % 64 || p.Cout % 32) return TL_ERR_UNSUPPORTED;
  const int64_t ld_b = p.in_ld * 2, in_bytes = (p.n_in - 1) * ld_b + (int64_t)p.Cin * 2;
  if (!(in_bytes > 0 && in_bytes + 2 * ld_b < 0xFFFFFFFFll)) return TL_ERR_UNSUPPORTED;
  const int nb = p.Cout / 32, pn = p.Cin / 64;
  if (p.K == 27) {
    if (nb == 2 && pn == 1) return launch<27, 2, 1, 2>(p, s);
    if (nb == 2 && pn == 2) return launch<27, 2, 2, 2>(p, s);
    if (nb == 4 && pn == 2) return launch<27, 4, 2, 2>(p, s);
    if (nb == 4 && pn == 1) return launch<27, 4, 1, 2>(p, s);
    if (nb == 3 && pn == 3) return launch<27, 3, 3, 2>(p, s);
    if (nb == 4 && pn == 4) return launch<27, 4, 2, 2, 8, 1, 2>(p, s);
  } else if (p.K == 8) {
    if (nb == 3 && pn == 1) return launch<8, 3, 1, 2>(p, s);
  }
  return TL_ERR_UNSUPPORTED;
}

#ifndef TL_F16_BUILD
int tl_launch_conv_streamq_x3(const ConvP& p, hipStream_t s) {
  if (!p.w_x3 || p.in_scale || p.in_relu || p.Cin % 32 || p.Cout % 32 || p.K != 27 || p.epi_mode != TL_EPI_NONE || p.Cin >= 256) return TL_ERR_UNSUPPORTED;
  const int64_t ld_b = p.in_ld * 4, in_bytes = (p.n_in - 1) * ld_b + (int64_t)p.Cin * 4;
  if (!(in_bytes > 0 && in_bytes + 2 * ld_b < 0xFFFFFFFFll) || ((uintptr_t)p.w_x3) % 16) return TL_ERR_UNSUPPORTED;
  const int nb = p.Cout / 32, pn = p.Cin / 32;
  if (nb == 2 && pn == 2) return launch<27, 2, 2, 1, 8, 1, 1, true, true>(p, s);
  if (nb == 2 && pn == 4) return launch<27, 2, 2, 1, 8, 1, 2, true>(p, s);
  if (nb == 3 && pn == 6) return launch<27, 3, 3, 2, 8, 1, 2, true>(p, s);
  return TL_ERR_UNSUPPORTED;
}
#endif
```

### treelearn_amd/csrc/tl_exec.hip

```cpp
#include <string.h>
#include <vector>

#include "tl_common.h"
#include "tl_arena.h"

namespace {

constexpr int64_t kCompactMinRows = 65536;
constexpr int64_t kBlkMinRows = 16384;
constexpr int64_t kBlkMaxRows = (1 << 25) - 64;
constexpr size_t kHostBytes = 64 + (size_t)TL_POINT_COORDS_MAX_PARTS * 16;

struct Ten {
  int64_t off = -1;
  int64_t ld = 0, n = 0;
  int C = 0;
  int64_t own_off = -1, own_bytes = 0;
};

struct ViewReq {
  const Ten* dst = nullptr;
  tl_affine aff{nullptr, nullptr};
  int relu = 0;
};

struct Table {
  const int32_t* table = nullptr;
  const int32_t* compact = nullptr;
  const int32_t* scatter = nullptr;
  bool blk = false;
  int one_hot = 0;
};

struct LevelG {
  int32_t dims[4];
  int64_t n = 0;
  int64_t coords = -1, nbr = -1, ct = -1, child = -1, inv = -1, invp = -1;
};

}

struct tl_exec {
  int32_t* host = nullptr;
  hipEvent_t ev_main = nullptr, ev_side = nullptr, ev_flag = nullptr;
  bool flag_in_flight = false;
  bool profile = false;
  std::vector<hipEvent_t> pev;
  std::vector<tl_launch_rec> recs;
  hipStream_t prof_stream = nullptr;
};

namespace {

struct Run {
  tl_exec* ex;
  const tl_net_desc* net;
  tl_forward_args* a;
  hipStream_t s;
  Arena ar;
  int esize;
  int rc = TL_OK;
  int launches = 0;
  int nl;
  LevelG lv[TL_MAX_LEVELS];
  bool blocked = false;
  int64_t g0 = 0;
  int64_t o_unit = -1, o_counter = -1, o_halo = -1, o_lrb = -1, o_pmask = -1, o_nn = -1;

  const int32_t* gw(int64_t word_off) const { return word_off < 0 ? nullptr : reinterpret_cast<const int32_t*>(ar.at(g0 + 4 * word_off)); }

  Ten alloc(int64_t n, int C) {
    Ten t;
    t.n = n; t.C = C; t.ld = C; t.own_bytes = n * C * esize; t.own_off = t.off = ar.take(t.own_bytes);
    return t;
  }
  void release(Ten& t) {
    if (t.own_off >= 0) ar.give(t.own_off, t.own_bytes);
    t.own_off = -1;
  }
  Ten cols(const Ten& t, int c0, int C) const {
    Ten v;
    v.off = t.off + (int64_t)c0 * esize; v.ld = t.ld; v.n = t.n; v.C = C;
    return v;
  }

  Table subm(int li) const {
    Table t;
    if (li == 0 && blocked) { t.blk = true; return t; }
    t.table = gw(lv[li].nbr); t.compact = gw(lv[li].ct);
    return t;
  }
  Table down(int li) const { Table t; t.table = gw(lv[li].child); return t; }
  Table up(int li) const {
    Table t;
    t.scatter = gw(lv[li].child);
    if (lv[li].invp >= 0) { t.table = gw(lv[li].invp); t.one_hot = 2; }
    else { t.table = gw(lv[li].inv); t.one_hot = 1; }
    return t;
  }

  void conv(int level, int kind, const Ten& x, const tl_weight& w, const Table& tb, int64_t n_out, const ViewReq* views, int nviews, Ten* outs,
            const Ten* residual = nullptr, tl_affine in_aff = {nullptr, nullptr}, int in_relu = 0, int all_ones = 0, int split_part = -1, int split_cin = 0) {
    for (int i = 0; i < nviews; ++i) outs[i] = views[i].dst ? *views[i].dst : alloc(n_out, w.Cout);
    if (rc != TL_OK) return;
    ++launches;
    if (ar.dry) return;
    tl_conv_args c{};
    c.in = ar.at(x.off); c.in_ld = x.ld; c.weight = w.w; c.weight_frag = w.frag; c.weight_x3 = w.x3;
    c.table = tb.table; c.table_compact = tb.compact; c.table_one_hot = tb.one_hot; c.table_scatter = tb.scatter;
    if (tb.blk) {
      c.blk_unit = gw(o_unit); c.blk_counter = gw(o_counter); c.blk_halo = gw(o_halo);
      c.blk_lrb = reinterpret_cast<const uint32_t*>(gw(o_lrb)); c.blk_pmask = gw(o_pmask);
    }
    c.in_all_ones = all_ones;
    c.n_out = n_out; c.n_in = x.n; c.K = w.K; c.Cin = w.Cin; c.Cout = w.Cout; c.dtype = net->dtype;
    c.in_scale = in_aff.scale; c.in_shift = in_aff.shift; c.in_relu = in_relu;
    if (residual) { c.residual = ar.at(residual->off); c.res_ld = residual->ld; }
    c.out = ar.at(outs[0].off); c.out_ld = outs[0].ld; c.out_scale = views[0].aff.scale; c.out_shift = views[0].aff.shift; c.out_relu = views[0].relu;
    if (nviews > 1) { c.out2 = ar.at(outs[1].off); c.out2_ld = outs[1].ld; c.out2_scale = views[1].aff.scale; c.out2_shift = views[1].aff.shift; c.out2_relu = views[1].relu; }
    if (nviews > 2) { c.out3 = ar.at(outs[2].off); c.out3_ld = outs[2].ld; c.out3_scale = views[2].aff.scale; c.out3_shift = views[2].aff.shift; c.out3_relu = views[2].relu; }
    const bool prof = ex->profile;
    if (prof) {
      hipEvent_t e0 = nullptr, e1 = nullptr;
      if (hipEventCreate(&e0) != hipSuccess || hipEventCreate(&e1) != hipSuccess) { rc = TL_ERR_LAUNCH; return; }
      ex->pev.push_back(e0); ex->pev.push_back(e1);
      tl_launch_rec r{};
      r.level = level; r.kind = kind; r.K = w.K; r.Cin = w.Cin; r.Cout = w.Cout; r.residual = residual != nullptr; r.esize = esize;
      r.split_part = split_part; r.split_cin = split_cin; r.in_prologue = in_aff.scale != nullptr || in_relu; r.n_out = n_out; r.n_in = x.n;
      ex->recs.push_back(r);
      if (hipEventRecord(e0, s) != hipSuccess) rc = TL_ERR_LAUNCH;
    }
    const int r = tl_conv_fwd(&c, s);
    if (prof && hipEventRecord(ex->pev.back(), s) != hipSuccess) rc = TL_ERR_LAUNCH;
    if (r != TL_OK) rc = r;
  }

  static ViewReq RAW(const Ten* dst = nullptr) { ViewReq v; v.dst = dst; return v; }
  static ViewReq ACT(const tl_affine& aff, const Ten* dst = nullptr) { ViewReq v; v.dst = dst; v.aff = aff; v.relu = 1; return v; }

  void res_block(int li, const tl_res_desc& b, const Ten& x_raw, const Ten& x_act, const ViewReq* views, int nviews, Ten* outs) {
    const Table nb = subm(li);
    const int64_t n = lv[li].n;
    Ten t, res;
    const ViewReq v1 = ACT(b.bn3);
    conv(li, 0, x_act, b.w1, nb, n, &v1, 1, &t);
    const bool has1x1 = b.w1x1.w != nullptr;
    if (has1x1) { const ViewReq vr = RAW(); conv(li, 3, x_raw, b.w1x1, Table{}, n, &vr, 1, &res); }
    conv(li, 0, t, b.w2, nb, n, views, nviews, outs, has1x1 ? &res : &x_raw);
    release(t);
    if (has1x1) release(res);
  }

  void ublock(int li, Ten x_raw, Ten x_act, const ViewReq* views, int nviews, Ten* outs) {
    const tl_ublock_desc& u = net->u[li];
    const int64_t n = lv[li].n;
    const int C = u.C;
    Ten o2[3];
    { const ViewReq v[2] = {RAW(), ACT(u.blocks[1].bn0)}; res_block(li, u.blocks[0], x_raw, x_act, v, 2, o2); }
    release(x_raw); release(x_act);
    x_raw = o2[0]; x_act = o2[1];
    if (!u.deeper) {
      res_block(li, u.blocks[1], x_raw, x_act, views, nviews, outs);
      release(x_raw); release(x_act);
      return;
    }
    Ten cat_raw = alloc(n, 2 * C), cat_act = alloc(n, 2 * C);
    const Ten cr_l = cols(cat_raw, 0, C), cr_r = cols(cat_raw, C, C), ca_l = cols(cat_act, 0, C), ca_r = cols(cat_act, C, C);
    Ten o3[3];
    { const ViewReq v[3] = {RAW(&cr_l), ACT(u.bn_cat_l, &ca_l), ACT(u.bn_down)}; res_block(li, u.blocks[1], x_raw, x_act, v, 3, o3); }
    release(x_raw); release(x_act);
    Ten xd = o3[2], d[2];
    { const ViewReq v[2] = {RAW(), ACT(net->u[li + 1].blocks[0].bn0)}; conv(li, 1, xd, u.wd, down(li), lv[li + 1].n, v, 2, d); }
    release(xd);
    Ten e_act;
    { const ViewReq v = ACT(u.bn_up); ublock(li + 1, d[0], d[1], &v, 1, &e_act); }
    { const ViewReq v[2] = {RAW(&cr_r), ACT(u.bn_cat_r, &ca_r)}; Ten o[2]; conv(li, 2, e_act, u.wu, up(li), n, v, 2, o); }
    release(e_act);
    Ten y[2];
    { const ViewReq v[2] = {RAW(), ACT(u.tail[1].bn0)}; res_block(li, u.tail[0], cat_raw, cat_act, v, 2, y); }
    release(cat_raw); release(cat_act);
    res_block(li, u.tail[1], y[0], y[1], views, nviews, outs);
    release(y[0]); release(y[1]);
  }

  void l1_block(const tl_res_desc& b, const Ten& x, const tl_affine& in_aff, const ViewReq* views, int nviews, Ten* outs) {
    const Table nb = subm(0);
    const int64_t n = lv[0].n;
    Ten t, res;
    const ViewReq v1 = ACT(b.bn3);
    conv(0, 0, x, b.w1, nb, n, &v1, 1, &t, nullptr, in_aff, 1);
    const bool has1x1 = b.w1x1.w != nullptr;
    if (has1x1) { const ViewReq vr = RAW(); conv(0, 3, x, b.w1x1, Table{}, n, &vr, 1, &res); }
    conv(0, 0, t, b.w2, nb, n, views, nviews, outs, has1x1 ? &res : &x);
    release(t);
    if (has1x1) release(res);
  }
  void l1_staged(Ten x_raw, const ViewReq* views, int nviews, Ten* outs) {
    const tl_ublock_desc& u = net->u[0];
    const int64_t n = lv[0].n;
    const int C = u.C;
    const Table nb = subm(0);
    Ten x1;
    { const ViewReq v = RAW(); l1_block(u.blocks[0], x_raw, u.blocks[0].bn0, &v, 1, &x1); }
    release(x_raw);
    Ten cat_raw = alloc(n, 2 * C);
    const Ten cr_l = cols(cat_raw, 0, C), cr_r = cols(cat_raw, C, C);
    Ten o2[2];
    { const ViewReq v[2] = {RAW(&cr_l), ACT(u.bn_down)}; l1_block(u.blocks[1], x1, u.blocks[1].bn0, v, 2, o2); }
    release(x1);
    Ten xd = o2[1], d[2];
    { const ViewReq v[2] = {RAW(), ACT(net->u[1].blocks[0].bn0)}; conv(0, 1, xd, u.wd, down(0), lv[1].n, v, 2, d); }
    release(xd);
    Ten e_act;
    { const ViewReq v = ACT(u.bn_up); ublock(1, d[0], d[1], &v, 1, &e_act); }
    { const ViewReq v = RAW(&cr_r); Ten o; conv(0, 2, e_act, u.wu, up(0), n, &v, 1, &o); }
    release(e_act);
    const tl_res_desc& b = u.tail[0];
    Ten part, t, res, y;
    { const ViewReq v = RAW(); conv(0, 0, cr_l, b.w1_half[0], nb, n, &v, 1, &part, nullptr, u.bn_cat_l, 1, 0, 0, 2 * C); }
    { const ViewReq v = ACT(b.bn3); conv(0, 0, cr_r, b.w1_half[1], nb, n, &v, 1, &t, &part, u.bn_cat_r, 1, 0, 1, 2 * C); }
    release(part);
    { const ViewReq v = RAW(); conv(0, 3, cat_raw, b.w1x1, Table{}, n, &v, 1, &res); }
    { const ViewReq v = RAW(); conv(0, 0, t, b.w2, nb, n, &v, 1, &y, &res); }
    release(t); release(res); release(cat_raw);
    l1_block(u.tail[1], y, u.tail[1].bn0, views, nviews, outs);
    release(y);
  }

  void network() {
    const int64_t n1 = lv[0].n;
    const bool feats = net->use_coords || net->use_feats;
    Ten ones = alloc(n1, net->in_channels);
    if (feats) {
      const int64_t ws_bytes = 4 * n1 * net->max_points_per_voxel, o_ws = ar.take(ws_bytes);
      if (!ar.dry) {
        const int r = tl_voxel_feats(a->xyz, a->point_feats, net->in_channels - 3, reinterpret_cast<const int64_t*>(gw(o_v2p)), a->N, n1, net->max_points_per_voxel,
                                     net->use_coords, net->use_feats, net->dtype, reinterpret_cast<int32_t*>(ar.at(o_ws)), ar.at(ones.off), s);
        if (r != TL_OK) rc = r;
      }
      ar.give(o_ws, ws_bytes);
    } else if (!ar.dry) {
      hipError_t e;
      if (net->dtype == TL_F32) e = hipMemsetD32Async((hipDeviceptr_t)ar.at(ones.off), 0x3F800000, n1 * net->in_channels, s);
      else e = hipMemsetD16Async((hipDeviceptr_t)ar.at(ones.off), net->dtype == TL_BF16 ? 0x3F80 : 0x3C00, n1 * net->in_channels, s);
      if (e != hipSuccess) rc = TL_ERR_LAUNCH;
    }
    Ten xs[2], x;
    const ViewReq out = RAW();
    if (blocked) {
      const ViewReq v = RAW();
      Table tin = subm(0);
      if (feats) { tin = Table{}; tin.table = gw(o_nn); }
      conv(0, 4, ones, net->w_in, tin, n1, &v, 1, xs, nullptr, {nullptr, nullptr}, 0, feats ? 0 : 1);
      release(ones);
      l1_staged(xs[0], &out, 1, &x);
    } else {
      const ViewReq v[2] = {RAW(), ACT(net->u[0].blocks[0].bn0)};
      conv(0, 4, ones, net->w_in, subm(0), n1, v, 2, xs, nullptr, {nullptr, nullptr}, 0, feats ? 0 : 1);
      release(ones);
      ublock(0, xs[0], xs[1], &out, 1, &x);
    }
    if (rc == TL_OK && !ar.dry) {
      const int r = tl_head_mlp(ar.at(x.off), x.ld, net->dtype, x.C, reinterpret_cast<const int64_t*>(gw(o_v2p)), a->N, net->out_bn.scale, net->out_bn.shift,
                                net->head_w1, net->head_b1, net->head_w2, net->head_b2, a->backbone, a->logits, a->offsets, s);
      if (r != TL_OK) rc = r;
    }
    release(x);
  }
  int64_t o_v2p = -1;
};

inline int64_t al64(int64_t w) { return (w + 63) & ~int64_t(63); }

inline bool weight_is(const tl_weight& w, int K, int Cin, int Cout) { return w.w && w.K == K && w.Cin == Cin && w.Cout == Cout; }
inline bool affine_ok(const tl_affine& a) { return a.scale && a.shift; }

inline bool res_ok(const tl_res_desc& b, int Cin, int C) {
  if (!affine_ok(b.bn0) || !affine_ok(b.bn3) || !weight_is(b.w1, 27, Cin, C) || !weight_is(b.w2, 27, C, C)) return false;
  if (Cin != C ? !weight_is(b.w1x1, 1, Cin, C) : b.w1x1.w != nullptr) return false;
  for (int h = 0; h < 2; ++h)
    if (b.w1_half[h].w && !(Cin == 2 * C && weight_is(b.w1_half[h], 27, C, C))) return false;
  return (b.w1_half[0].w == nullptr) == (b.w1_half[1].w == nullptr);
}

inline bool net_ok(const tl_net_desc* net) {
  const int nl = net->num_levels;
  if (!weight_is(net->w_in, 27, net->in_channels, net->u[0].C)) return false;
  if (net->u[0].C != 8 && net->u[0].C != 16 && net->u[0].C != 32 && net->u[0].C != 64) return false;
  if (!affine_ok(net->out_bn) || !net->head_w1 || !net->head_b1 || !net->head_w2 || !net->head_b2) return false;
  for (int l = 0; l < nl; ++l) {
    const tl_ublock_desc& u = net->u[l];
    if (u.C <= 0 || (u.deeper != 0) != (l + 1 < nl)) return false;
    if (!res_ok(u.blocks[0], u.C, u.C) || !res_ok(u.blocks[1], u.C, u.C)) return false;
    if (!u.deeper) continue;
    const int Cd = net->u[l + 1].C;
    if (!affine_ok(u.bn_down) || !affine_ok(u.bn_up) || !affine_ok(u.bn_cat_l) || !affine_ok(u.bn_cat_r)) return false;
    if (!weight_is(u.wd, 8, u.C, Cd) || !weight_is(u.wu, 8, Cd, u.C)) return false;
    if (!res_ok(u.tail[0], 2 * u.C, u.C) || !res_ok(u.tail[1], u.C, u.C)) return false;
  }
  return true;
}

}

extern "C" {

tl_exec* tl_exec_create(void) {
  tl_exec* ex = new (std::nothrow) tl_exec();
  if (!ex) return nullptr;
  if (hipHostMalloc(reinterpret_cast<void**>(&ex->host), kHostBytes, hipHostMallocDefault) != hipSuccess || (memset(ex->host, 0, kHostBytes), false) ||
      hipEventCreateWithFlags(&ex->ev_main, hipEventDisableTiming) != hipSuccess || hipEventCreateWithFlags(&ex->ev_side, hipEventDisableTiming) != hipSuccess ||
      hipEventCreateWithFlags(&ex->ev_flag, hipEventDisableTiming) != hipSuccess) {
    tl_exec_destroy(ex);
    return nullptr;
  }
  return ex;
}

void tl_exec_destroy(tl_exec* ex) {
  if (!ex) return;
  for (hipEvent_t e : ex->pev) (void)hipEventDestroy(e);
  if (ex->ev_main) (void)hipEventDestroy(ex->ev_main);
  if (ex->ev_side) (void)hipEventDestroy(ex->ev_side);
  if (ex->ev_flag) (void)hipEventDestroy(ex->ev_flag);
  if (ex->host) (void)hipHostFree(ex->host);
  delete ex;
}

int tl_exec_check(tl_exec* ex) {
  if (!ex) return TL_ERR_ARG;
  if (ex->flag_in_flight) {
    if (hipEventSynchronize(ex->ev_flag) != hipSuccess) return TL_ERR_LAUNCH;
    ex->flag_in_flight = false;
  }
  if (ex->host[8]) {
    ex->host[8] = 0;
    return TL_ERR_BLK;
  }
  return TL_OK;
}

int tl_exec_profile(tl_exec* ex, int enable) {
  if (!ex) return TL_ERR_ARG;
  ex->profile = enable != 0;
  return TL_OK;
}

int tl_exec_profile_read(tl_exec* ex, tl_launch_rec* recs, int cap) {
  if (!ex || !recs || cap < 0) return TL_ERR_ARG;
  const int n = (int)ex->recs.size();
  if (n == 0) return 0;
  if (hipEventSynchronize(ex->pev.back()) != hipSuccess) return TL_ERR_LAUNCH;
  for (int i = 0; i < n && i < cap; ++i) {
    recs[i] = ex->recs[i];
    if (hipEventElapsedTime(&recs[i].ms, ex->pev[2 * i], ex->pev[2 * i + 1]) != hipSuccess) return TL_ERR_LAUNCH;
  }
  return n < cap ? n : cap;
}

int tl_forward(tl_exec* ex, const tl_net_desc* net, tl_forward_args* a, tl_stream_t stream) {
  if (!ex || !net || !a || !a->xyz || !a->batch_ids || !a->logits || !a->offsets || a->N <= 0 || a->B <= 0) return TL_ERR_ARG;
  if (net->num_levels < 2 || net->num_levels > TL_MAX_LEVELS || net->in_channels <= 0 || net->voxel_size <= 0.f) return TL_ERR_ARG;
  if (net->dtype != TL_F32 && net->dtype != TL_BF16 && net->dtype != TL_F16) return TL_ERR_ARG;
  if (!net_ok(net)) return TL_ERR_ARG;
  const bool feats = net->use_coords || net->use_feats;
  if (feats && (!a->point_feats || net->in_channels <= 3 || net->in_channels > 8 || net->max_points_per_voxel <= 0)) return TL_ERR_ARG;
  if (!a->arena || ((uintptr_t)a->arena) % 256) return TL_ERR_ARG;
  hipStream_t s = tl_s(stream);
  const int nl = net->num_levels;
  const int64_t N = a->N;
  a->needed_bytes = 0; a->blocked_used = 0; a->launches = 0;
  for (hipEvent_t e : ex->pev) (void)hipEventDestroy(e);
  ex->pev.clear(); ex->recs.clear();

  Run R;
  R.ex = ex; R.net = net; R.a = a; R.s = s; R.nl = nl;
  R.esize = net->dtype == TL_F32 ? 4 : 2;
  R.ar.base = static_cast<char*>(a->arena); R.ar.cap = a->arena_bytes; R.ar.dry = false;

  const bool one = a->B == 1;
  const int64_t o_pc = R.ar.take(16 * N), o_maxc = R.ar.take(one ? 16 * TL_POINT_COORDS_MAX_PARTS : 16), o_mm = R.ar.take(one ? 24 * 256 : 24 * (int64_t)a->B);
  if (R.ar.peak > R.ar.cap) { a->needed_bytes = R.ar.peak * 3; return TL_ERR_ARENA; }
  int32_t* pcoords = reinterpret_cast<int32_t*>(R.ar.at(o_pc));
  int rc, n_parts = 0;
  if (one) rc = tl_voxel_point_coords_one(a->xyz, a->batch_ids, N, net->voxel_size, reinterpret_cast<uint32_t*>(R.ar.at(o_mm)), pcoords,
                                          reinterpret_cast<int32_t*>(R.ar.at(o_maxc)), &n_parts, stream);
  else rc = tl_voxel_point_coords(a->xyz, a->batch_ids, N, a->B, net->voxel_size, reinterpret_cast<uint32_t*>(R.ar.at(o_mm)), pcoords,
                                  reinterpret_cast<int32_t*>(R.ar.at(o_maxc)), stream);
  if (rc != TL_OK) return rc;
  if (one) {
    if (hipMemcpyAsync(ex->host + 16, R.ar.at(o_maxc), 16 * (size_t)n_parts, hipMemcpyDeviceToHost, s) != hipSuccess || hipStreamSynchronize(s) != hipSuccess) return TL_ERR_LAUNCH;
    for (int j = 0; j < 4; ++j) ex->host[j] = 0;
    for (int q = 0; q < n_parts; ++q)
      for (int j = 0; j < 4; ++j) ex->host[j] = ex->host[j] > ex->host[16 + 4 * q + j] ? ex->host[j] : ex->host[16 + 4 * q + j];
  } else if (hipMemcpyAsync(ex->host, R.ar.at(o_maxc), 16, hipMemcpyDeviceToHost, s) != hipSuccess || hipStreamSynchronize(s) != hipSuccess) return TL_ERR_LAUNCH;
  ex->flag_in_flight = false;
  if (ex->host[3]) return TL_ERR_EXTENT;
  if (ex->host[8]) {
    ex->host[8] = 0;
    return TL_ERR_BLK;
  }
  const int32_t extent[3] = {ex->host[0] + 1, ex->host[1] + 1, ex->host[2] + 1};
  int32_t shape[TL_MAX_LEVELS][3];
  for (int j = 0; j < 3; ++j) {
    shape[0][j] = net->has_shape ? net->spatial_shape[j] : extent[j];
    if (extent[j] > shape[0][j]) return TL_ERR_EXTENT;
  }
  for (int l = 1; l < nl; ++l)
    for (int j = 0; j < 3; ++j) {
      shape[l][j] = shape[l - 1][j] / 2;
      if (shape[l][j] <= 0) return TL_ERR_REACH_ZERO;
    }

  int64_t nw[TL_MAX_LEVELS], woff[TL_MAX_LEVELS + 1];
  {
    int32_t d[4] = {a->B, extent[0], extent[1], extent[2]};
    woff[0] = 0;
    for (int l = 0; l < nl; ++l) {
      for (int j = 0; j < 4; ++j) R.lv[l].dims[j] = d[j];
      nw[l] = tl_nwords(tl_dims(d));
      woff[l + 1] = woff[l] + nw[l];
      for (int j = 1; j < 4; ++j) d[j] = (d[j] + 1) / 2;
    }
  }
  const int64_t tw = woff[nl];
  const int64_t n_ws = tl_pyramid_ws_words(R.lv[0].dims, nl, nullptr);
  if (n_ws < 0) return TL_ERR_ARG;
  const int64_t o_pyr = R.ar.take(4 * (3 * tw + 8 + n_ws));
  if (R.ar.peak > R.ar.cap) { a->needed_bytes = R.ar.peak * 2; return TL_ERR_ARENA; }
  char* p0 = R.ar.at(o_pyr);
  rc = tl_pyramid_build(pcoords, N, R.lv[0].dims, shape[0], nl, reinterpret_cast<uint64_t*>(p0), reinterpret_cast<uint32_t*>(p0 + 8 * tw),
                        reinterpret_cast<uint32_t*>(p0 + 12 * tw), reinterpret_cast<uint32_t*>(p0 + 12 * tw + 32), stream);
  if (rc != TL_OK) return rc;
  if (hipMemcpyAsync(ex->host, p0 + 12 * tw, 4 * nl, hipMemcpyDeviceToHost, s) != hipSuccess || hipStreamSynchronize(s) != hipSuccess) return TL_ERR_LAUNCH;
  for (int l = 0; l < nl; ++l) {
    R.lv[l].n = a->level_n[l] = (int64_t)(uint32_t)ex->host[l];
    if (R.lv[l].n <= 0) return TL_ERR_REACH_ZERO;
  }

  const int64_t n1 = R.lv[0].n;
  const tl_ublock_desc& u0 = net->u[0];
  const bool x3_l1 = u0.blocks[0].w1.x3 && u0.blocks[0].w2.x3 && u0.blocks[1].w1.x3 && u0.blocks[1].w2.x3 && u0.tail[0].w1_half[0].x3 && u0.tail[0].w1_half[1].x3 &&
                     u0.tail[0].w2.x3 && u0.tail[1].w1.x3 && u0.tail[1].w2.x3;
  R.blocked = net->blocked && (net->dtype != TL_F32 || x3_l1) && u0.C == 32 && u0.deeper && u0.tail[0].w1_half[0].w && u0.tail[0].w1_half[1].w &&
              n1 >= kBlkMinRows && n1 <= kBlkMaxRows;
  a->blocked_used = R.blocked;
  int64_t cur = 0;
  auto take = [&](int64_t words) { const int64_t o = cur; cur += al64(words); return o; };
  R.o_v2p = take(2 * N);
  for (int l = 0; l < nl; ++l) {
    LevelG& v = R.lv[l];
    const bool skip = R.blocked && l == 0;
    if (!skip) { v.coords = take(4 * v.n); v.nbr = take(27 * v.n); }
    if (!skip && v.n >= kCompactMinRows) v.ct = take(10 * v.n);
    if (l + 1 < nl) v.child = take(8 * R.lv[l + 1].n);
  }
  int64_t o_o2n = -1, o_perm = -1, o_cnew = -1, o_bws = -1;
  if (R.blocked) {
    const int64_t nbws = tl_blk_ws_words(R.lv[0].dims);
    o_o2n = take(n1); o_perm = take(n1); o_cnew = take(4 * n1); R.o_unit = take(4 * n1); R.o_counter = take(64); R.o_halo = take(32 * n1);
    R.o_lrb = take(9 * n1); R.o_pmask = take(n1); o_bws = take(nbws);
    if (feats) R.o_nn = take(27 * n1);
  }
  const bool packed0 = nl > 1 && net->u[0].C == 32 && net->u[1].C == 64 && (net->dtype != TL_F32 || net->u[0].wu.x3) && tl_conv_one_hot_direct_enabled(n1);
  const int64_t o_m1 = cur;
  for (int l = 0; l + 1 < nl; ++l) {
    if (l == 0 && packed0) R.lv[l].invp = take(R.lv[l].n);
    else R.lv[l].inv = take(8 * R.lv[l].n);
  }
  const int64_t o_m1_end = cur;
  R.g0 = R.ar.take(4 * cur);

  {
    Run D = R;
    D.ar.dry = true; D.ar.base = nullptr;
    D.network();
    a->needed_bytes = D.ar.peak;
    if (D.ar.peak > R.ar.cap) return TL_ERR_ARENA;
  }

  auto W = [&](int64_t word_off) { return word_off < 0 ? nullptr : reinterpret_cast<int32_t*>(R.ar.at(R.g0 + 4 * word_off)); };
  tl_level arr[TL_MAX_LEVELS];
  for (int l = 0; l < nl; ++l) {
    LevelG& v = R.lv[l];
    tl_level& t = arr[l];
    for (int j = 0; j < 4; ++j) t.dims[j] = v.dims[j];
    t.n = v.n;
    t.bitmap = reinterpret_cast<const uint64_t*>(p0 + 8 * woff[l]); t.prefix = reinterpret_cast<const uint32_t*>(p0 + 8 * tw + 4 * woff[l]);
    t.coords = W(v.coords); t.nbr = W(v.nbr); t.compact = W(v.ct); t.child = W(v.child); t.parent = nullptr; t.inv = W(v.inv); t.inv_packed = W(v.invp); t.o2n = nullptr;
  }
  hipStream_t side = s;
  struct Join {
    tl_exec* ex; hipStream_t s; hipStream_t* side; bool done = false;
    int join() {
      if (done || *side == s) return TL_OK;
      done = true;
      return (hipEventRecord(ex->ev_side, *side) == hipSuccess && hipStreamWaitEvent(s, ex->ev_side, 0) == hipSuccess) ? TL_OK : TL_ERR_LAUNCH;
    }
    ~Join() { (void)join(); }
  } joiner{ex, s, &side};
  if (R.blocked) {
    tl_blk bk{};
    bk.o2n = W(o_o2n); bk.perm = W(o_perm); bk.coords_new = W(o_cnew); bk.unit = W(R.o_unit); bk.counter = W(R.o_counter); bk.halo = W(R.o_halo);
    bk.lrb = reinterpret_cast<uint32_t*>(W(R.o_lrb)); bk.pmask = W(R.o_pmask); bk.cap_units = n1; bk.halo_max = TL_BLK_HALO_MAX; bk.nn = W(R.o_nn);
    rc = tl_blk_build(arr[0].bitmap, arr[0].prefix, R.lv[0].dims, n1, &bk, reinterpret_cast<uint32_t*>(W(o_bws)), 1, stream);
    if (rc != TL_OK) return rc;
    arr[0].o2n = bk.o2n;
    if (a->side_stream && tl_s(a->side_stream) != s) {
      side = tl_s(a->side_stream);
      if (hipEventRecord(ex->ev_main, s) != hipSuccess || hipStreamWaitEvent(side, ex->ev_main, 0) != hipSuccess) return TL_ERR_LAUNCH;
    }
    rc = tl_blk_build(arr[0].bitmap, arr[0].prefix, R.lv[0].dims, n1, &bk, reinterpret_cast<uint32_t*>(W(o_bws)), 2, reinterpret_cast<tl_stream_t>(side));
    if (rc != TL_OK) return rc;
  }
  rc = tl_rulebooks_build(arr, nl, W(o_m1), o_m1_end - o_m1, pcoords, N, reinterpret_cast<int64_t*>(W(R.o_v2p)), stream);
  if (rc != TL_OK) return rc;
  if (joiner.join() != TL_OK) return TL_ERR_LAUNCH;
  if (R.blocked) {
    if (hipMemcpyAsync(ex->host + 8, W(R.o_counter) + 1, 4, hipMemcpyDeviceToHost, s) != hipSuccess || hipEventRecord(ex->ev_flag, s) != hipSuccess) return TL_ERR_LAUNCH;
    ex->flag_in_flight = true;
  }

  R.network();
  a->launches = R.launches;
  return R.rc;
}

}
```

### treelearn_amd/csrc/tl_voxel.hip

```cpp
#include "tl_common.h"

namespace {

constexpr int kBlock = 256;

__device__ __forceinline__ uint32_t enc_f32(float f) {
  uint32_t u = __float_as_uint(f);
  return u ^ ((u >> 31) ? 0xFFFFFFFFu : 0x80000000u);
}
__device__ __forceinline__ float dec_f32(uint32_t u) {
  return __uint_as_float((u & 0x80000000u) ? (u ^ 0x80000000u) : ~u);
}

__global__ void k_init_minmax(uint32_t* __restrict__ mm, int B, int32_t* __restrict__ maxc) {
  const int i = blockIdx.x * blockDim.x + threadIdx.x;
  if (i < B * 6) mm[i] = ((i % 6) < 3) ? 0xFFFFFFFFu : 0u;
  if (i < 4) maxc[i] = 0;
}

__global__ void __launch_bounds__(kBlock) k_minmax(const float* __restrict__ xyz, const int64_t* __restrict__ bid,
                                                   int64_t N_all, int B, uint32_t* __restrict__ mm) {
  uint32_t lo[3] = {0xFFFFFFFFu, 0xFFFFFFFFu, 0xFFFFFFFFu}, hi[3] = {0u, 0u, 0u};
  int cb = -1;
  auto flush = [&]() {
// ... 403 lines not shown
      uint32_t inc = v;
      for (int off = 1; off < 64; off <<= 1) {
        const uint32_t t = (uint32_t)__shfl_up((int)inc, off);
        if (lane >= off) inc += t;
      }
      if (lane == 63) wsum[wid] = inc;
      __syncthreads();
      uint32_t before = 0, tot = 0;
      for (int w = 0; w < kPyrBlock / 64; ++w) { if (w < wid) before += wsum[w]; tot += wsum[w]; }
      __syncthreads();
      if (i < n) prefix[i] = carry + before + inc - v;
      carry += tot;
    }
    if (threadIdx.x == 0) counts[p.first + j] = carry;
    __threadfence_block();
    __syncthreads();
  }
}

__device__ __forceinline__ void expand_coords_body(const uint64_t* __restrict__ bm, const uint32_t* __restrict__ pf, const TlDims& d,
                                                   int32_t* __restrict__ coords, int64_t first, int64_t stride) {
  const int64_t n = tl_nwords(d);
  for (int64_t i = first; i < n; i += stride) {
    uint64_t w = bm[i];
    if (!w) continue;
    const int zw = (int)(i % d.Zw);
    int64_t r = i / d.Zw;
    const int y = (int)(r % d.Y); r /= d.Y;
    const int x = (int)(r % d.X);
    const int b = (int)(r / d.X);
    int64_t row = pf[i];
    while (w) {
      const int bit = __ffsll((unsigned long long)w) - 1;
      reinterpret_cast<int4*>(coords)[row++] = make_int4(b, x, y, zw * 64 + bit);
      w &= w - 1;
    }
  }
}

__global__ void __launch_bounds__(kBlock) k_expand_coords(const uint64_t* __restrict__ bm, const uint32_t* __restrict__ pf, TlDims d,
                                                          int32_t* __restrict__ coords) {
  expand_coords_body(bm, pf, d, coords, (int64_t)blockIdx.x * blockDim.x + threadIdx.x, (int64_t)gridDim.x * blockDim.x);
}

__global__ void __launch_bounds__(kBlock) k_point_rank(const int32_t* __restrict__ pc, int64_t N, const uint64_t* __restrict__ bm,
                                                       const uint32_t* __restrict__ pf, TlDims d, int64_t* __restrict__ v2p,
                                                       const int32_t* __restrict__ o2n) {
  for (int64_t i = (int64_t)blockIdx.x * blockDim.x + threadIdx.x; i < N; i += (int64_t)gridDim.x * blockDim.x) {
    const int4 c = reinterpret_cast<const int4*>(pc)[i];
    int r = -1;
    if (c.x >= 0 && c.x < d.B && c.y < d.X && c.z < d.Y && c.w < d.Z) r = tl_rank_at(bm, pf, tl_col_word(d, c.x, c.y, c.z), c.w);
    if (o2n && r >= 0) r = o2n[r];
    v2p[i] = r;
  }
}

__device__ __forceinline__ void rulebook_subm_body(const int32_t* __restrict__ coords, int64_t M, const uint64_t* __restrict__ bm,
                                                   const uint32_t* __restrict__ pf, const TlDims& d, int32_t* __restrict__ nbr,
                                                   int32_t* __restrict__ compact, int64_t first, int64_t stride) {
  for (int64_t i = first; i < M; i += stride) {
    const int4 c = reinterpret_cast<const int4*>(coords)[i];
    uint32_t cmask = 0;
#pragma unroll
    for (int dx = -1; dx <= 1; ++dx) {
#pragma unroll
      for (int dy = -1; dy <= 1; ++dy) {
        const int x = c.y + dx, y = c.z + dy;
        const int tap0 = (dx + 1) * 9 + (dy + 1) * 3;
        int r0 = -1, r1 = -1, r2 = -1;
        if (x >= 0 && x < d.X && y >= 0 && y < d.Y) {
          const int64_t wc = tl_col_word(d, c.x, x, y);
          const int z = c.w;
          const int64_t w = wc + (z >> 6);
          const uint64_t word = bm[w];
          const uint32_t base = pf[w];
          const int bit = z & 63;
          const uint64_t below = (1ull << bit) - 1;
          if (word & (1ull << bit)) r1 = (int)(base + __popcll(word & below));
          if (bit > 0) { if (word & (1ull << (bit - 1))) r0 = (int)(base + __popcll(word & (below >> 1))); }
          else if (z > 0) r0 = tl_rank_at(bm, pf, wc, z - 1);
          if (bit < 63) { if (word & (2ull << bit)) r2 = (int)(base + __popcll(word & ((below << 1) | 1ull))); }
          else if (z + 1 < d.Z) r2 = tl_rank_at(bm, pf, wc, z + 1);
        }
        nbr[(int64_t)(tap0 + 0) * M + i] = r0;
        nbr[(int64_t)(tap0 + 1) * M + i] = r1;
        nbr[(int64_t)(tap0 + 2) * M + i] = r2;
        if (compact) {
          compact[(int64_t)(tap0 / 3) * M + i] = r0 >= 0 ? r0 : (r1 >= 0 ? r1 : r2);
          cmask |= ((r0 >= 0 ? 1u : 0u) | (r1 >= 0 ? 2u : 0u) | (r2 >= 0 ? 4u : 0u)) << tap0;
        }
      }
    }
    if (compact) compact[(int64_t)9 * M + i] = (int32_t)cmask;
  }
}

__global__ void __launch_bounds__(kBlock) k_rulebook_subm(const int32_t* __restrict__ coords, int64_t M, const uint64_t* __restrict__ bm,
                                                          const uint32_t* __restrict__ pf, TlDims d, int32_t* __restrict__ nbr,
                                                          int32_t* __restrict__ compact) {
  rulebook_subm_body(coords, M, bm, pf, d, nbr, compact, (int64_t)blockIdx.x * blockDim.x + threadIdx.x, (int64_t)gridDim.x * blockDim.x);
}

__device__ __forceinline__ void rulebook_down_body(const int32_t* __restrict__ cc, int64_t Mc, const uint64_t* __restrict__ fbm,
                                                   const uint32_t* __restrict__ fpf, const TlDims& f, int64_t Mf, int32_t* __restrict__ child,
                                                   int32_t* __restrict__ parent, int32_t* __restrict__ inv, int64_t first, int64_t stride,
                                                   const int32_t* __restrict__ fo2n = nullptr, int32_t* __restrict__ invp = nullptr) {
  for (int64_t q = first; q < Mc; q += stride) {
    const int4 c = reinterpret_cast<const int4*>(cc)[q];
#pragma unroll
    for (int k = 0; k < 8; ++k) {
      const int x = 2 * c.y + (k >> 2), y = 2 * c.z + ((k >> 1) & 1), z = 2 * c.w + (k & 1);
      int r = -1;
      if (x < f.X && y < f.Y && z < f.Z) r = tl_rank_at(fbm, fpf, tl_col_word(f, c.x, x, y), z);
      if (fo2n && r >= 0) r = fo2n[r];
      child[(int64_t)k * Mc + q] = r;
      if (r >= 0) {
        if (parent) parent[r] = (int)q;
        if (inv) inv[(int64_t)k * Mf + r] = (int)q;
        if (invp) invp[r] = (int)((q << 3) | k);
      }
    }
  }
}

__global__ void __launch_bounds__(kBlock) k_rulebook_down(const int32_t* __restrict__ cc, int64_t Mc, const uint64_t* __restrict__ fbm,
                                                          const uint32_t* __restrict__ fpf, TlDims f, int64_t Mf,
                                                          int32_t* __restrict__ child, int32_t* __restrict__ parent, int32_t* __restrict__ inv,
                                                          const int32_t* __restrict__ fo2n, int32_t* __restrict__ invp) {
  rulebook_down_body(cc, Mc, fbm, fpf, f, Mf, child, parent, inv, (int64_t)blockIdx.x * blockDim.x + threadIdx.x, (int64_t)gridDim.x * blockDim.x, fo2n, invp);
}

struct LevelPack {
  int nl;
  int first[kPyrMaxLevels + 1];
  TlDims d[kPyrMaxLevels];
  int64_t n[kPyrMaxLevels];
  const uint64_t* bm[kPyrMaxLevels];
  const uint32_t* pf[kPyrMaxLevels];
  int32_t* coords[kPyrMaxLevels];
  int32_t* nbr[kPyrMaxLevels];
  int32_t* child[kPyrMaxLevels];
  int32_t* parent[kPyrMaxLevels];
  int32_t* inv[kPyrMaxLevels];
};
__device__ __forceinline__ int pack_level(const LevelPack& p) {
  int l = 0;
  while (l + 1 < p.nl && (int)blockIdx.x >= p.first[l + 1]) ++l;
  return l;
}
__global__ void __launch_bounds__(kBlock) k_expand_coords_multi(LevelPack p) {
  const int l = pack_level(p);
  expand_coords_body(p.bm[l], p.pf[l], p.d[l], p.coords[l], (int64_t)(blockIdx.x - p.first[l]) * kBlock + threadIdx.x,
                     (int64_t)(p.first[l + 1] - p.first[l]) * kBlock);
}
__global__ void __launch_bounds__(kBlock) k_rulebook_subm_multi(LevelPack p) {
  const int l = pack_level(p);
  rulebook_subm_body(p.coords[l], p.n[l], p.bm[l], p.pf[l], p.d[l], p.nbr[l], nullptr,
                     (int64_t)(blockIdx.x - p.first[l]) * kBlock + threadIdx.x, (int64_t)(p.first[l + 1] - p.first[l]) * kBlock);
}
__global__ void __launch_bounds__(kBlock) k_rulebook_down_multi(LevelPack p) {
  const int l = pack_level(p);
  rulebook_down_body(p.coords[l + 1], p.n[l + 1], p.bm[l], p.pf[l], p.d[l], p.n[l], p.child[l], p.parent[l], p.inv[l],
                     (int64_t)(blockIdx.x - p.first[l]) * kBlock + threadIdx.x, (int64_t)(p.first[l + 1] - p.first[l]) * kBlock);
}

__global__ void __launch_bounds__(kBlock) k_table_compact(const int32_t* __restrict__ t, int64_t n, int32_t* __restrict__ o) {
  for (int64_t r = (int64_t)blockIdx.x * blockDim.x + threadIdx.x; r < n; r += (int64_t)gridDim.x * blockDim.x) {
    uint32_t mask = 0;
    for (int c = 0; c < 9; ++c) {
// ... 188 lines not shown
  TL_CHECK_LAUNCH();
  return TL_OK;
}

int64_t tl_pyramid_ws_words(const int32_t dims0[4], int num_levels, int64_t* level_word_offsets) {
  if (!dims0 || num_levels < 1 || num_levels > kPyrMaxLevels) return -1;
  int32_t d[4] = {dims0[0], dims0[1], dims0[2], dims0[3]};
  int64_t off = 0, ws = 0;
  for (int l = 0; l < num_levels; ++l) {
    const int64_t nw = tl_nwords(tl_dims(d));
    if (level_word_offsets) level_word_offsets[l] = off;
    off += nw;
    ws += tl_scan_ws_words(nw);
    for (int j = 1; j < 4; ++j) d[j] = (d[j] + 1) / 2;
  }
  if (level_word_offsets) level_word_offsets[num_levels] = off;
  {
    int32_t d0[4] = {dims0[0], dims0[1], dims0[2], dims0[3]};
    ws += 4 + 16 * tl_nwords(tl_dims(d0));
  }
  return ws;
}

int tl_pyramid_build(const int32_t* pcoords, int64_t N, const int32_t dims0[4], const int32_t shape0[3], int num_levels,
                     uint64_t* bitmaps, uint32_t* prefixes, uint32_t* counts, uint32_t* ws, tl_stream_t stream) {
  if (!pcoords || !dims0 || !shape0 || !bitmaps || !prefixes || !counts || !ws || N <= 0 || num_levels < 1 || num_levels > kPyrMaxLevels)
    return TL_ERR_ARG;
  hipStream_t s = tl_s(stream);
  TlDims d[kPyrMaxLevels];
  int out[kPyrMaxLevels][3];
  int64_t off[kPyrMaxLevels + 1];
  int32_t dd[4] = {dims0[0], dims0[1], dims0[2], dims0[3]};
  int sh[3] = {shape0[0], shape0[1], shape0[2]};
  off[0] = 0;
  for (int l = 0; l < num_levels; ++l) {
    d[l] = tl_dims(dd);
    for (int j = 0; j < 3; ++j) out[l][j] = sh[j];
    off[l + 1] = off[l] + tl_nwords(d[l]);
    for (int j = 1; j < 4; ++j) dd[j] = (dd[j] + 1) / 2;
    for (int j = 0; j < 3; ++j) sh[j] /= 2;
  }
  {
    int64_t scan_ws = 0;
    for (int l2 = 0; l2 < num_levels; ++l2) scan_ws += tl_scan_ws_words(tl_nwords(d[l2]));
    uint8_t* bytes = reinterpret_cast<uint8_t*>((reinterpret_cast<uintptr_t>(ws + scan_ws) + 15) & ~uintptr_t(15));
    const int64_t nw0 = tl_nwords(d[0]);
    if (hipMemsetAsync(bytes, 0, nw0 * 64, s) != hipSuccess) return TL_ERR_LAUNCH;
    k_set_bytes<<<tl_grid(N, kBlock), kBlock, 0, s>>>(pcoords, N, d[0], bytes);
    k_bytes_to_bits<<<tl_grid(nw0, kBlock), kBlock, 0, s>>>(bytes, nw0, bitmaps);
  }
  int l = 0;
  ScanPack sp;
  sp.first[0] = 0;
  for (; l < num_levels; ++l) {
    const int64_t nw = tl_nwords(d[l]);
    if (l > 0 && nw <= kPyrSmallWords) break;
    if (l > 0)
      k_bitmap_down<<<tl_grid(nw, kBlock), kBlock, 0, s>>>(bitmaps + off[l - 1], d[l - 1], out[l][0], out[l][1], out[l][2], bitmaps + off[l], d[l]);
    sp.off[l] = off[l]; sp.nw[l] = nw; sp.first[l + 1] = sp.first[l] + (int)tl_cdiv(nw, kScanTile);
  }
  sp.nl = l;
  k_scan_partials_multi<<<(unsigned)sp.first[l], kBlock, 0, s>>>(bitmaps, sp, ws);
  k_scan_blocks_multi<<<1, kBlock, 0, s>>>(ws, sp, counts);
  k_scan_final_multi<<<(unsigned)sp.first[l], kBlock, 0, s>>>(bitmaps, sp, ws, prefixes);
  if (l < num_levels) {
    PyrSmall p;
    p.nl = num_levels - l; p.first = l;
    p.d[0] = d[l - 1]; p.off[0] = off[l - 1];
    for (int j = 0; j < p.nl; ++j) {
      p.d[j + 1] = d[l + j]; p.off[j + 1] = off[l + j];
      for (int k = 0; k < 3; ++k) p.out[j][k] = out[l + j][k];
    }
    k_pyramid_small<<<1, kPyrBlock, 0, s>>>(bitmaps, prefixes, counts, p);
  }
  TL_CHECK_LAUNCH();
  return TL_OK;
}

int tl_rulebooks_build(const tl_level* lv, int num_levels, int32_t* minus_one, int64_t minus_one_words,
                       const int32_t* pcoords, int64_t N, int64_t* v2p, tl_stream_t stream) {
  if (!lv || num_levels < 1 || num_levels > kPyrMaxLevels) return TL_ERR_ARG;
  for (int l = 0; l < num_levels; ++l) {
    if (!lv[l].bitmap || !lv[l].prefix || lv[l].n <= 0) return TL_ERR_ARG;
    if ((!lv[l].coords || !lv[l].nbr) && !lv[l].o2n) return TL_ERR_ARG;
    if (lv[l].nbr && !lv[l].coords) return TL_ERR_ARG;
    if (l > 0 && !lv[l].coords) return TL_ERR_ARG;
    if (l + 1 < num_levels && (!lv[l].child || (!lv[l].inv && !lv[l].inv_packed))) return TL_ERR_ARG;
    if (lv[l].inv_packed && lv[l].n >= (1ll << 28)) return TL_ERR_ARG;
  }
  hipStream_t s = tl_s(stream);
  auto inside = [&](const int32_t* q, int64_t words) { return minus_one && q >= minus_one && q + words <= minus_one + minus_one_words; };
  if (minus_one && minus_one_words > 0 && hipMemsetAsync(minus_one, 0xFF, minus_one_words * 4, s) != hipSuccess) return TL_ERR_LAUNCH;
  for (int l = 0; l + 1 < num_levels; ++l) {
    if (lv[l].parent && !inside(lv[l].parent, lv[l].n) && hipMemsetAsync(lv[l].parent, 0xFF, lv[l].n * 4, s) != hipSuccess) return TL_ERR_LAUNCH;
    if (lv[l].inv && !inside(lv[l].inv, lv[l].n * 8) && hipMemsetAsync(lv[l].inv, 0xFF, lv[l].n * 32, s) != hipSuccess) return TL_ERR_LAUNCH;
    if (lv[l].inv_packed && !inside(lv[l].inv_packed, lv[l].n) && hipMemsetAsync(lv[l].inv_packed, 0xFF, lv[l].n * 4, s) != hipSuccess) return TL_ERR_LAUNCH;
  }
  int small = num_levels;
  for (int l = num_levels - 1; l >= 1; --l) {
    if (tl_nwords(tl_dims(lv[l].dims)) <= kPyrSmallWords && lv[l].n <= 64 * kPyrSmallWords && !lv[l].compact && !lv[l].o2n && !lv[l - 1].o2n &&
        !lv[l].inv_packed && !lv[l - 1].inv_packed) small = l; else break;
  }
  if (num_levels - small < 2) small = num_levels;
  for (int l = 0; l < small; ++l) {
    const TlDims d = tl_dims(lv[l].dims);
    if (lv[l].coords) k_expand_coords<<<tl_grid(tl_nwords(d), kBlock), kBlock, 0, s>>>(lv[l].bitmap, lv[l].prefix, d, lv[l].coords);
    if (lv[l].nbr) k_rulebook_subm<<<tl_grid(lv[l].n, kBlock), kBlock, 0, s>>>(lv[l].coords, lv[l].n, lv[l].bitmap, lv[l].prefix, d, lv[l].nbr, lv[l].compact);
  }
  LevelPack p;
  p.nl = num_levels - small;
  if (p.nl > 0) {
    for (int j = 0; j < p.nl; ++j) {
      const tl_level& v = lv[small + j];
      p.d[j] = tl_dims(v.dims); p.n[j] = v.n; p.bm[j] = v.bitmap; p.pf[j] = v.prefix; p.coords[j] = v.coords; p.nbr[j] = v.nbr;
      p.child[j] = v.child; p.parent[j] = v.parent; p.inv[j] = v.inv;
    }
    p.first[0] = 0;
    for (int j = 0; j < p.nl; ++j) p.first[j + 1] = p.first[j] + (int)tl_cdiv(tl_nwords(p.d[j]), kBlock);
    k_expand_coords_multi<<<p.first[p.nl], kBlock, 0, s>>>(p);
    for (int j = 0; j < p.nl; ++j) p.first[j + 1] = p.first[j] + (int)tl_cdiv(p.n[j], kBlock);
    k_rulebook_subm_multi<<<p.first[p.nl], kBlock, 0, s>>>(p);
  }
  for (int l = 0; l + 1 < num_levels && l < small; ++l) {
    const tl_level &f = lv[l], &c = lv[l + 1];
    k_rulebook_down<<<tl_grid(c.n, kBlock), kBlock, 0, s>>>(c.coords, c.n, f.bitmap, f.prefix, tl_dims(f.dims), f.n, f.child, f.parent, f.inv, f.o2n, f.inv_packed);
  }
  if (p.nl > 1) {
    p.nl -= 1;
    for (int j = 0; j < p.nl; ++j) p.first[j + 1] = p.first[j] + (int)tl_cdiv(p.n[j + 1], kBlock);
    k_rulebook_down_multi<<<p.first[p.nl], kBlock, 0, s>>>(p);
  }
  if (v2p) {
    if (!pcoords || N <= 0) return TL_ERR_ARG;
    k_point_rank<<<tl_grid(N, kBlock), kBlock, 0, s>>>(pcoords, N, lv[0].bitmap, lv[0].prefix, tl_dims(lv[0].dims), v2p, lv[0].o2n);
  }
  TL_CHECK_LAUNCH();
  return TL_OK;
}

int tl_rulebook_compact(const int32_t* table, int64_t n, int32_t* compact, tl_stream_t stream) {
  if (!table || !compact || n <= 0) return TL_ERR_ARG;
  k_table_compact<<<tl_grid(n, kBlock), kBlock, 0, tl_s(stream)>>>(table, n, compact);
  TL_CHECK_LAUNCH();
  return TL_OK;
}

}
```

### treelearn_amd/model/executor.py

```python
import collections
import contextlib
import ctypes
import os
import threading

import torch

from .. import _hip, ops

MAX_CONTEXTS = int(os.environ.get("TL_EXEC_MAX_CONTEXTS", "8"))
_ENV_DEFAULTS = (("TL_BLK_PRO", "1"), ("TL_NO_ONES_TABLE", "0"), ("TL_NO_COMPACT", "0"), ("TL_EXEC", "1"))
KINDS = ("subm", "down", "inverse", "1x1", "input")


def _aff(dst, pair):
    dst.scale = pair[0].data_ptr(); dst.shift = pair[1].data_ptr()


def _wt(dst, w):
    if w is None:
        return
    dst.w = w.data_ptr(); dst.frag = _hip.ptr(getattr(w, "_tl_frag", None)); dst.x3 = _hip.ptr(getattr(w, "_tl_x3", None))
    dst.K, dst.Cout, dst.Cin = w.shape

# ... 152 lines not shown

    def check(self, dev=None, stream=None):
        if stream is not None:
            dev = dev or torch.device("cuda", torch.cuda.current_device())
        with self._pinned(dev, stream) as ctxs:
            for c in ctxs:
                with c.lock:
                    self._raise_if_flagged(_hip.lib().tl_exec_check(c.handle))

    def profile(self, enable):
        self.profiling = bool(enable)
        with self._pinned() as ctxs:
            for c in ctxs:
                with c.lock:
                    _hip.lib().tl_exec_profile(c.handle, int(self.profiling))

    def profile_read(self, dev=None, stream=None):
        stream = stream or torch.cuda.current_stream()
        dev = dev or torch.device("cuda", torch.cuda.current_device())
        buf = (_hip.LaunchRec * 512)()
        with self._pinned(dev, stream, create=True) as (ctx,), ctx.lock:
            n = _hip.lib().tl_exec_profile_read(ctx.handle, buf, 512)
        if n < 0:
            _hip.check(n, "tl_exec_profile_read")
        out = []
        for r in buf[:n]:
            out.append(dict(level=r.level, kind=KINDS[r.kind], K=r.K, Cin=r.Cin, Cout=r.Cout, n_out=r.n_out, n_in=r.n_in, residual=bool(r.residual),
                            esize=r.esize, split=(r.split_part, r.split_cin) if r.split_part >= 0 else None, in_scale=bool(r.in_prologue), ms=r.ms))
        return out

    def forward(self, coords, batch_ids, batch_size, want_backbone=True, input_feats=None):
        L = _hip.lib()
        _hip.require_cuda(coords, "coords"); _hip.require_cuda(batch_ids, "batch_ids")
        if coords.dtype != torch.float32 or batch_ids.dtype != torch.int64:
            raise TypeError("coords must be float32 [N,3] and batch_ids int64 [N]")
        N = coords.shape[0]
        if self.needs_feats:
            if input_feats is None:
                raise ValueError("this network reads point features (use_coords / use_feats): pass input_feats")
            _hip.require_cuda(input_feats, "input_feats")
            if input_feats.dtype != torch.float32 or not input_feats.is_contiguous() or tuple(input_feats.shape) != (N, self.desc.in_channels - 3):
                raise TypeError(f"input_feats must be contiguous float32 [N, {self.desc.in_channels - 3}]")
        if N == 0:
            raise ValueError("empty tile")
        dev = coords.device
        stream = torch.cuda.current_stream(dev)
        with self._pinned(dev, stream, create=True) as (ctx,):
            if self.profiling:
                L.tl_exec_profile(ctx.handle, 1)
            plan = self._plan_ref()
            if plan is None:
                raise RuntimeError("the InferencePlan of this executor is gone")
            self.desc.blocked = int(plan.supports_blocked())
            bb = torch.empty((N, self.head_C), dtype=torch.float32, device=dev) if want_backbone else None
            logits = torch.empty((N, 2), dtype=torch.float32, device=dev)
            offsets = torch.empty((N, 3), dtype=torch.float32, device=dev)
            a = _hip.ForwardArgs()
            a.xyz = coords.data_ptr(); a.batch_ids = batch_ids.data_ptr(); a.N = N; a.B = int(batch_size)
            a.backbone = _hip.ptr(bb); a.logits = logits.data_ptr(); a.offsets = offsets.data_ptr()
            a.point_feats = input_feats.data_ptr() if self.needs_feats else None
            if stream == torch.cuda.default_stream(dev):
                from ..geometry import _side_stream
                a.side_stream = _side_stream(dev).cuda_stream
            with ctx.lock:
                for attempt in range(4):
                    if ctx.arena is None:
                        ctx.new_arena(max(1 << 20, int(N * 1536)))
                    a.arena = ctx.arena.data_ptr(); a.arena_bytes = ctx.arena.numel()
                    rc = L.tl_forward(ctx.handle, ctypes.byref(self.desc), ctypes.byref(a), stream.cuda_stream)
                    if rc != _hip.TL_ERR_ARENA:
                        break
                    ctx.new_arena(int(a.needed_bytes * 1.15) + (1 << 20))
                if rc == _hip.TL_OK and ctx.arena.numel() > 4 * int(a.needed_bytes) + (64 << 20):
                    ctx.drop_arena()
                if rc == _hip.TL_OK and os.environ.get("TL_EXEC_CHECK") == "1":
                    rc = L.tl_exec_check(ctx.handle)
        if rc == _hip.TL_ERR_BLK:
            self._raise_if_flagged(rc)
        if rc == _hip.TL_ERR_REACH_ZERO:
            raise ValueError("sparse conv output spatial shape reach zero!!! (a level of the tile is empty or its spatial shape collapsed)")
        if rc == _hip.TL_ERR_EXTENT:
            raise ValueError("voxelize: tile extent exceeds spatial_shape, batch id out of range or voxel coordinate outside [0, 65536)")
        _hip.check(rc, "tl_forward")
        self.last = dict(level_n=list(a.level_n[:self.desc.num_levels]), blocked=bool(a.blocked_used), launches=a.launches, arena_bytes=a.needed_bytes)
        return bb, logits, offsets
```

Before: 257.6 Mpoints/s.

## Skip full 27-tap neighbor tables for levels whose convs use compact tables

```diff
diff --git a/include/treelearn_hip.h b/include/treelearn_hip.h
--- a/include/treelearn_hip.h
+++ b/include/treelearn_hip.h
@@ -124,6 +124,7 @@
 int64_t tl_conv_red_parts(int64_t n_out);
 
 int tl_conv_fwd(const tl_conv_args* args, tl_stream_t stream);
+int tl_conv_fwd_probe(const tl_conv_args* args);
 
 int tl_pack_weight(const float* w_ref, int Cout, int K, int Cin, void* w_packed, int dtype, tl_stream_t stream);
 int64_t tl_pack_weight_x3_bytes(int Cout, int K, int Cin);
@@ -331,7 +332,8 @@
   float ms;
 } tl_launch_rec;
 typedef struct tl_forward_args {
-  const float* xyz; const int64_t* batch_ids; int64_t N; int32_t B; int32_t reserved;
+  const float* xyz; const int64_t* batch_ids; int64_t N; int32_t B;
+  int32_t lean_levels;
   const float* point_feats;
   void* arena; int64_t arena_bytes;
   float* backbone;
diff --git a/treelearn_amd/_hip.py b/treelearn_amd/_hip.py
--- a/treelearn_amd/_hip.py
+++ b/treelearn_amd/_hip.py
@@ -83,7 +83,7 @@
 
 
 class ForwardArgs(_c.Structure):
-    _fields_ = [("xyz", _vp), ("batch_ids", _vp), ("N", _i64), ("B", _i32), ("reserved", _i32), ("point_feats", _vp), ("arena", _vp), ("arena_bytes", _i64),
+    _fields_ = [("xyz", _vp), ("batch_ids", _vp), ("N", _i64), ("B", _i32), ("lean_levels", _i32), ("point_feats", _vp), ("arena", _vp), ("arena_bytes", _i64),
                 ("backbone", _vp), ("logits", _vp), ("offsets", _vp), ("side_stream", _vp), ("needed_bytes", _i64),
                 ("level_n", _i64 * TL_MAX_LEVELS), ("blocked_used", _i32), ("launches", _i32)]
 
@@ -114,6 +114,7 @@
     "tl_blk_ws_words": (_i64, [_I4]),
     "tl_blk_build": (_i32, [_vp, _vp, _I4, _i64, _c.POINTER(Blk), _vp, _i32, _vp]),
     "tl_conv_fwd": (_i32, [_c.POINTER(ConvArgs), _vp]),
+    "tl_conv_fwd_probe": (_i32, [_c.POINTER(ConvArgs)]),
     "tl_conv_red_parts": (_i64, [_i64]),
     "tl_exec_create": (_vp, []),
     "tl_exec_destroy": (None, [_vp]),
diff --git a/treelearn_amd/csrc/tl_common.h b/treelearn_amd/csrc/tl_common.h
--- a/treelearn_amd/csrc/tl_common.h
+++ b/treelearn_amd/csrc/tl_common.h
@@ -56,4 +56,5 @@
   return (int)(pf[w] + __popcll(word & (bit - 1)));
 }
 
+bool tl_forward_lean_enabled();
 bool tl_conv_one_hot_direct_enabled(int64_t n_out);
diff --git a/treelearn_amd/csrc/tl_conv.hip b/treelearn_amd/csrc/tl_conv.hip
--- a/treelearn_amd/csrc/tl_conv.hip
+++ b/treelearn_amd/csrc/tl_conv.hip
@@ -343,6 +343,9 @@
 static int g_blk = 1;
 static int g_up = 1;
 
+static int g_lean_geometry = 1;
+bool tl_forward_lean_enabled() { return g_lean_geometry != 0; }
+
 bool tl_conv_one_hot_direct_enabled(int64_t n_out) { return g_direct && g_direct_oh && n_out > g_small_rows; }
 
 extern "C" {
@@ -356,6 +359,7 @@
   if (!strcmp(key, "stream")) { g_stream = (int)value; return TL_OK; }
   if (!strcmp(key, "streamq")) { g_streamq = (int)value; return TL_OK; }
   if (!strcmp(key, "streamq_x3")) { if (value != 0 && value != 1) return TL_ERR_ARG; g_streamq_x3 = (int)value; return TL_OK; }
+  if (!strcmp(key, "lean_geometry")) { if (value != 0 && value != 1) return TL_ERR_ARG; g_lean_geometry = (int)value; return TL_OK; }
   if (!strcmp(key, "small_rows")) { g_small_rows = value; return TL_OK; }
   if (!strcmp(key, "small_mode")) { g_small_mode = (int)value; return TL_OK; }
   if (!strcmp(key, "wgrad_dense")) { g_wgrad_dense = (int)value; return TL_OK; }
@@ -365,10 +369,12 @@
   return TL_ERR_ARG;
 }
 
-int tl_conv_fwd(const tl_conv_args* a, tl_stream_t stream) {
+static int conv_fwd_dispatch(const tl_conv_args* a, tl_stream_t stream, bool probe) {
   if (!a || !a->in || !a->weight || !a->out || a->n_out <= 0 || a->K <= 0 || a->K > 27 || a->Cin <= 0 || a->Cout <= 0) return TL_ERR_ARG;
   const bool has_blk = a->blk_unit && a->blk_counter && a->blk_halo && a->blk_lrb && a->K == 27;
-  if (!a->table && a->K != 1 && !has_blk && !(a->in_all_ones && a->blk_pmask)) return TL_ERR_ARG;
+  const bool lean = a->K == 27 && !a->table && a->table_compact && !has_blk;
+  if (probe && !lean) return TL_ERR_ARG;
+  if (!a->table && a->K != 1 && !has_blk && !(a->in_all_ones && a->blk_pmask) && !lean) return TL_ERR_ARG;
   if ((a->in_scale == nullptr) != (a->in_shift == nullptr)) return TL_ERR_ARG;
   if ((a->out_scale == nullptr) != (a->out_shift == nullptr)) return TL_ERR_ARG;
   if (a->dtype != TL_F32 && a->dtype != TL_BF16 && a->dtype != TL_F16) return TL_ERR_ARG;
@@ -397,6 +403,7 @@
   p.blk_pmask = a->K == 27 ? a->blk_pmask : nullptr;
   p.epi_mode = a->epi_mode; p.red_part = a->red_part; p.red_nparts = a->red_nparts; p.bn_x = a->bn_x; p.bn_x_ld = a->bn_x_ld;
   p.bn_mean = a->bn_mean; p.bn_rstd = a->bn_rstd; p.bn_scale = a->bn_scale; p.bn_shift = a->bn_shift; p.bn_relu = a->bn_relu;
+  p.probe = probe;
   const bool train = a->epi_mode != TL_EPI_NONE;
   if (train) {
     if ((a->epi_mode != TL_EPI_STATS && a->epi_mode != TL_EPI_BN_BWD) || !a->red_part || ((uintptr_t)a->red_part) % 8) return TL_ERR_ARG;
@@ -417,7 +424,7 @@
   const bool vec_ok = (a->in_ld % 8 == 0) && (((uintptr_t)a->in) % 16 == 0) && (((uintptr_t)a->weight) % 16 == 0);
   const bool out_vec = (a->out_ld % 8 == 0) && (((uintptr_t)a->out) % 16 == 0) &&
                        (!a->out2 || (a->out2_ld % 8 == 0 && ((uintptr_t)a->out2) % 16 == 0)) && (!a->out3 || (a->out3_ld % 8 == 0 && ((uintptr_t)a->out3) % 16 == 0));
-  if (a->in_all_ones && !train && (dt == TL_BF16 || (dt == TL_F32 && !f16)) && out_vec && (g_direct || !a->table) && ((uintptr_t)a->weight) % 4 == 0 && !a->residual) {
+  if (a->in_all_ones && !train && (dt == TL_BF16 || (dt == TL_F32 && !f16)) && out_vec && (g_direct || (!a->table && !lean)) && ((uintptr_t)a->weight) % 4 == 0 && !a->residual) {
     const int rc = L_ones27(p, dt, s);
     if (rc != TL_ERR_UNSUPPORTED) return rc;
   }
@@ -430,7 +437,7 @@
     const int rc = tl_launch_conv_blk_x3(p, s);
     if (rc != TL_ERR_UNSUPPORTED) return rc;
   }
-  if (!a->table && a->K != 1) return TL_ERR_UNSUPPORTED;
+  if (!a->table && a->K != 1 && !lean) return TL_ERR_UNSUPPORTED;
   if (a->table_scatter && p.one_hot && g_up && !train && dt == TL_BF16 && vec_ok && out_vec &&
       (!a->out_scale || (((uintptr_t)a->out_scale) % 16 == 0 && ((uintptr_t)a->out_shift) % 16 == 0))) {
     const int rc = L_up(p, a->table_scatter, s);
@@ -438,11 +445,12 @@
   }
   if (dt == TL_BF16 && a->Cin == 4 && a->Cout == 32 && g_direct && out_vec && ((uintptr_t)a->in) % 8 == 0 && ((uintptr_t)a->weight) % 16 == 0 &&
       (!a->residual || (a->res_ld % 8 == 0 && ((uintptr_t)a->residual) % 16 == 0))) {
+    if (lean) return TL_CONV_NEEDS_TABLE;
     const int rc = L_direct(p, TL_BF16, s);
     if (rc != TL_ERR_UNSUPPORTED) return rc;
   }
-  if (!train && a->Cin <= 8 && a->Cout % 8 == 0 && a->Cout <= 64 && !a->in_scale && !a->in_relu && out_vec) return L_tinycin(p, dt, s);
-  if (!train && vec_ok && a->n_out <= g_small_rows && a->Cin % 32 == 0 && a->Cout % 32 == 0) return L_small(p, dt, s);
+  if (!train && a->Cin <= 8 && a->Cout % 8 == 0 && a->Cout <= 64 && !a->in_scale && !a->in_relu && out_vec) return lean ? TL_CONV_NEEDS_TABLE : L_tinycin(p, dt, s);
+  if (!train && vec_ok && a->n_out <= g_small_rows && a->Cin % 32 == 0 && a->Cout % 32 == 0) return lean ? TL_CONV_NEEDS_TABLE : L_small(p, dt, s);
   if (train && a->n_out <= g_small_rows) return TL_ERR_UNSUPPORTED;
   const bool aligned = (a->in_ld % 4 == 0) && (((uintptr_t)a->in) % 16 == 0) && (((uintptr_t)a->weight) % 16 == 0) &&
                        (!a->in_scale || (((uintptr_t)a->in_scale) % 16 == 0 && ((uintptr_t)a->in_shift) % 16 == 0));
@@ -474,6 +482,7 @@
     if (g_stream) { const int rc = L_stream(p, TL_F32, s); if (rc != TL_ERR_UNSUPPORTED) return rc; }
   }
   if (train && dt == TL_F32) return TL_ERR_UNSUPPORTED;
+  if (lean && dt == TL_F32) return TL_CONV_NEEDS_TABLE;
   if (dt == TL_F32 && !f16 && vec_ok && a->n_out <= 4 * g_small_rows && a->Cin % 32 == 0 && a->Cout % 32 == 0 && !a->in_scale && !a->in_relu)
     return L_small(p, dt, s);
   if (dt == TL_F32 && aligned && a->Cin % KC == 0 && a->Cout % 32 == 0 && a->Cout <= 224) {
@@ -512,9 +521,11 @@
       if (rc != TL_ERR_UNSUPPORTED) return rc;
     }
     if (train) return TL_ERR_UNSUPPORTED;
+    if (lean) return TL_CONV_NEEDS_TABLE;
     return f16 ? tl_launch_conv_bf16_f16(p, s) : tl_launch_conv_bf16(p, s);
   }
   if (train || f16) return TL_ERR_UNSUPPORTED;
+  if (lean) return TL_CONV_NEEDS_TABLE;
   {
     const int rc = tl_launch_conv_tinycout(p, dt, s);
     if (rc != TL_ERR_UNSUPPORTED) return rc;
@@ -524,6 +535,16 @@
   else k_conv_generic<__hip_bfloat16><<<g, 256, 0, s>>>(p);
   TL_CHECK_LAUNCH();
   return TL_OK;
+}
+
+int tl_conv_fwd(const tl_conv_args* a, tl_stream_t stream) {
+  const int rc = conv_fwd_dispatch(a, stream, false);
+  return rc == TL_CONV_NEEDS_TABLE ? TL_ERR_UNSUPPORTED : rc;
+}
+
+int tl_conv_fwd_probe(const tl_conv_args* a) {
+  const int rc = conv_fwd_dispatch(a, nullptr, true);
+  return rc == TL_CONV_NEEDS_TABLE ? TL_ERR_UNSUPPORTED : rc;
 }
 
 int64_t tl_conv_red_parts(int64_t n_out) {
diff --git a/treelearn_amd/csrc/tl_conv_direct.hip b/treelearn_amd/csrc/tl_conv_direct.hip
--- a/treelearn_amd/csrc/tl_conv_direct.hip
+++ b/treelearn_amd/csrc/tl_conv_direct.hip
@@ -438,6 +438,10 @@
   constexpr int UB = BF16 ? 64 : 128;
   const size_t lds = (size_t)K * UN * NB * 32 * UB + (size_t)WAVES * 32 * (NB * 32 + 4) * 4 + (TR ? (size_t)WAVES * 2 * NB * 32 * 8 : 0);
   if (lds > 160 * 1024) return TL_ERR_UNSUPPORTED;
+  if constexpr (K != 1 && !CT) {
+    if (!p.table) return TL_CONV_NEEDS_TABLE;
+  }
+  if (p.probe) return TL_OK;
   static TlAttrOnce attr_once;
   if (!tl_lds_attr(attr_once, reinterpret_cast<const void*>(&k_conv_direct<BF16, K, NB, UN, G, WAVES, CT, TR, OH, X3>), 160 * 1024)) return TL_ERR_LAUNCH;
   const int ntiles = (int)tl_cdiv(p.n_out, 32);
@@ -494,6 +498,7 @@
 
 int tl_launch_conv_ones27(const ConvP& p, int dtype, hipStream_t s) {
   if (p.K != 27 || p.Cout != 32 || (!p.ctab && !p.blk_pmask) || p.Cin <= 0 || p.Cin > 64 || p.in_scale || p.in_relu || p.epi_mode != TL_EPI_NONE) return TL_ERR_UNSUPPORTED;
+  if (p.probe) return TL_OK;
   if (dtype == TL_BF16) k_conv_ones27<true><<<tl_grid(p.n_out * 4, 256), 256, 0, s>>>(p);
   else k_conv_ones27<false><<<tl_grid(p.n_out * 4, 256), 256, 0, s>>>(p);
   return hipGetLastError() == hipSuccess ? TL_OK : TL_ERR_LAUNCH;
diff --git a/treelearn_amd/csrc/tl_conv_internal.h b/treelearn_amd/csrc/tl_conv_internal.h
--- a/treelearn_amd/csrc/tl_conv_internal.h
+++ b/treelearn_amd/csrc/tl_conv_internal.h
@@ -44,7 +44,10 @@
   const float* bn_mean; const float* bn_rstd; const float* bn_scale; const float* bn_shift; int bn_relu;
   int one_hot;
   const int32_t* blk_unit; const int32_t* blk_counter; const int32_t* blk_halo; const uint32_t* blk_lrb; const int32_t* blk_pmask;
+  int probe;
 };
+
+constexpr int TL_CONV_NEEDS_TABLE = -1000;
 
 static __device__ __forceinline__ float ld_elem(const float* p) { return *p; }
 static __device__ __forceinline__ float ld_elem(const __hip_bfloat16* p) { return h16_lo((uint32_t)*reinterpret_cast<const uint16_t*>(p)); }
diff --git a/treelearn_amd/csrc/tl_conv_stream.hip b/treelearn_amd/csrc/tl_conv_stream.hip
--- a/treelearn_amd/csrc/tl_conv_stream.hip
+++ b/treelearn_amd/csrc/tl_conv_stream.hip
@@ -203,6 +203,7 @@
   const size_t wt = 2 * (size_t)NB * 32 * (UN * 32 * EB + 16), ep = (size_t)WAVES * 32 * 36 * 4;
   const size_t lds = wt > ep ? wt : ep;
   if (lds > 160 * 1024) return TL_ERR_UNSUPPORTED;
+  if (p.probe) return TL_OK;
   static TlAttrOnce attr_once;
   if (!tl_lds_attr(attr_once, reinterpret_cast<const void*>(&k_conv_stream<BF16, K, NB, UN, DA, RB, OCC, OH, X3>), 160 * 1024)) return TL_ERR_LAUNCH;
   p.nblk = (int)tl_cdiv(p.n_out, WAVES * 32 * RB);
diff --git a/treelearn_amd/csrc/tl_conv_streamq.hip b/treelearn_amd/csrc/tl_conv_streamq.hip
--- a/treelearn_amd/csrc/tl_conv_streamq.hip
+++ b/treelearn_amd/csrc/tl_conv_streamq.hip
@@ -258,6 +258,7 @@
   const size_t wt = 2 * (size_t)NB * 32 * (PN * 128 + 16) + (size_t)W * K * 32 * RB * 4, ep = (size_t)W * 32 * 36 * 4;
   const size_t lds = wt > ep ? wt : ep;
   if (lds > 160 * 1024) return TL_ERR_UNSUPPORTED;
+  if (p.probe) return TL_OK;
   static TlAttrOnce attr_once;
   if (!tl_lds_attr(attr_once, reinterpret_cast<const void*>(&k_conv_streamq<K, NB, PN, DA, W, RB, OCC, SP, X3, UL>), 160 * 1024)) return TL_ERR_LAUNCH;
   p.nblk = (int)tl_cdiv(p.n_out, W * 32 * RB);
diff --git a/treelearn_amd/csrc/tl_exec.hip b/treelearn_amd/csrc/tl_exec.hip
--- a/treelearn_amd/csrc/tl_exec.hip
+++ b/treelearn_amd/csrc/tl_exec.hip
@@ -64,9 +64,12 @@
   int nl;
   LevelG lv[TL_MAX_LEVELS];
   bool blocked = false;
+  bool probing = false;
+  uint32_t need_table = 0;
   int64_t g0 = 0;
   int64_t o_unit = -1, o_counter = -1, o_halo = -1, o_lrb = -1, o_pmask = -1, o_nn = -1;
 
+  bool live() const { return !ar.dry && !probing; }
   const int32_t* gw(int64_t word_off) const { return word_off < 0 ? nullptr : reinterpret_cast<const int32_t*>(ar.at(g0 + 4 * word_off)); }
 
   Ten alloc(int64_t n, int C) {
@@ -119,6 +122,13 @@
     c.out = ar.at(outs[0].off); c.out_ld = outs[0].ld; c.out_scale = views[0].aff.scale; c.out_shift = views[0].aff.shift; c.out_relu = views[0].relu;
     if (nviews > 1) { c.out2 = ar.at(outs[1].off); c.out2_ld = outs[1].ld; c.out2_scale = views[1].aff.scale; c.out2_shift = views[1].aff.shift; c.out2_relu = views[1].relu; }
     if (nviews > 2) { c.out3 = ar.at(outs[2].off); c.out3_ld = outs[2].ld; c.out3_scale = views[2].aff.scale; c.out3_shift = views[2].aff.shift; c.out3_relu = views[2].relu; }
+    if (probing) {
+      if (c.K == 27 && c.table && c.table_compact && !tb.blk) {
+        c.table = nullptr;
+        if (tl_conv_fwd_probe(&c) != TL_OK) need_table |= 1u << level;
+      }
+      return;
+    }
     const bool prof = ex->profile;
     if (prof) {
       hipEvent_t e0 = nullptr, e1 = nullptr;
@@ -233,13 +243,13 @@
     Ten ones = alloc(n1, net->in_channels);
     if (feats) {
       const int64_t ws_bytes = 4 * n1 * net->max_points_per_voxel, o_ws = ar.take(ws_bytes);
-      if (!ar.dry) {
+      if (live()) {
         const int r = tl_voxel_feats(a->xyz, a->point_feats, net->in_channels - 3, reinterpret_cast<const int64_t*>(gw(o_v2p)), a->N, n1, net->max_points_per_voxel,
                                      net->use_coords, net->use_feats, net->dtype, reinterpret_cast<int32_t*>(ar.at(o_ws)), ar.at(ones.off), s);
         if (r != TL_OK) rc = r;
       }
       ar.give(o_ws, ws_bytes);
-    } else if (!ar.dry) {
+    } else if (live()) {
       hipError_t e;
       if (net->dtype == TL_F32) e = hipMemsetD32Async((hipDeviceptr_t)ar.at(ones.off), 0x3F800000, n1 * net->in_channels, s);
       else e = hipMemsetD16Async((hipDeviceptr_t)ar.at(ones.off), net->dtype == TL_BF16 ? 0x3F80 : 0x3C00, n1 * net->in_channels, s);
@@ -260,7 +270,7 @@
       release(ones);
       ublock(0, xs[0], xs[1], &out, 1, &x);
     }
-    if (rc == TL_OK && !ar.dry) {
+    if (rc == TL_OK && live()) {
       const int r = tl_head_mlp(ar.at(x.off), x.ld, net->dtype, x.C, reinterpret_cast<const int64_t*>(gw(o_v2p)), a->N, net->out_bn.scale, net->out_bn.shift,
                                 net->head_w1, net->head_b1, net->head_w2, net->head_b2, a->backbone, a->logits, a->offsets, s);
       if (r != TL_OK) rc = r;
@@ -369,7 +379,7 @@
   hipStream_t s = tl_s(stream);
   const int nl = net->num_levels;
   const int64_t N = a->N;
-  a->needed_bytes = 0; a->blocked_used = 0; a->launches = 0;
+  a->needed_bytes = 0; a->blocked_used = 0; a->launches = 0; a->lean_levels = 0;
   for (hipEvent_t e : ex->pev) (void)hipEventDestroy(e);
   ex->pev.clear(); ex->recs.clear();
 
@@ -445,30 +455,46 @@
   R.blocked = net->blocked && (net->dtype != TL_F32 || x3_l1) && u0.C == 32 && u0.deeper && u0.tail[0].w1_half[0].w && u0.tail[0].w1_half[1].w &&
               n1 >= kBlkMinRows && n1 <= kBlkMaxRows;
   a->blocked_used = R.blocked;
-  int64_t cur = 0;
-  auto take = [&](int64_t words) { const int64_t o = cur; cur += al64(words); return o; };
-  R.o_v2p = take(2 * N);
-  for (int l = 0; l < nl; ++l) {
-    LevelG& v = R.lv[l];
-    const bool skip = R.blocked && l == 0;
-    if (!skip) { v.coords = take(4 * v.n); v.nbr = take(27 * v.n); }
-    if (!skip && v.n >= kCompactMinRows) v.ct = take(10 * v.n);
-    if (l + 1 < nl) v.child = take(8 * R.lv[l + 1].n);
-  }
-  int64_t o_o2n = -1, o_perm = -1, o_cnew = -1, o_bws = -1;
-  if (R.blocked) {
-    const int64_t nbws = tl_blk_ws_words(R.lv[0].dims);
-    o_o2n = take(n1); o_perm = take(n1); o_cnew = take(4 * n1); R.o_unit = take(4 * n1); R.o_counter = take(64); R.o_halo = take(32 * n1);
-    R.o_lrb = take(9 * n1); R.o_pmask = take(n1); o_bws = take(nbws);
-    if (feats) R.o_nn = take(27 * n1);
-  }
   const bool packed0 = nl > 1 && net->u[0].C == 32 && net->u[1].C == 64 && (net->dtype != TL_F32 || net->u[0].wu.x3) && tl_conv_one_hot_direct_enabled(n1);
-  const int64_t o_m1 = cur;
-  for (int l = 0; l + 1 < nl; ++l) {
-    if (l == 0 && packed0) R.lv[l].invp = take(R.lv[l].n);
-    else R.lv[l].inv = take(8 * R.lv[l].n);
-  }
-  const int64_t o_m1_end = cur;
+  int64_t cur = 0, o_o2n = -1, o_perm = -1, o_cnew = -1, o_bws = -1, o_m1 = 0, o_m1_end = 0;
+  auto layout = [&](uint32_t lean) {
+    cur = 0;
+    auto take = [&](int64_t words) { const int64_t o = cur; cur += al64(words); return o; };
+    R.o_v2p = take(2 * N);
+    for (int l = 0; l < nl; ++l) {
+      LevelG& v = R.lv[l];
+      const bool skip = R.blocked && l == 0;
+      v.coords = v.nbr = v.ct = v.child = v.inv = v.invp = -1;
+      if (!skip) { v.coords = take(4 * v.n); if (!(lean >> l & 1)) v.nbr = take(27 * v.n); }
+      if (!skip && v.n >= kCompactMinRows) v.ct = take(10 * v.n);
+      if (l + 1 < nl) v.child = take(8 * R.lv[l + 1].n);
+    }
+    if (R.blocked) {
+      const int64_t nbws = tl_blk_ws_words(R.lv[0].dims);
+      o_o2n = take(n1); o_perm = take(n1); o_cnew = take(4 * n1); R.o_unit = take(4 * n1); R.o_counter = take(64); R.o_halo = take(32 * n1);
+      R.o_lrb = take(9 * n1); R.o_pmask = take(n1); o_bws = take(nbws);
+      if (feats) R.o_nn = take(27 * n1);
+    }
+    o_m1 = cur;
+    for (int l = 0; l + 1 < nl; ++l) {
+      if (l == 0 && packed0) R.lv[l].invp = take(R.lv[l].n);
+      else R.lv[l].inv = take(8 * R.lv[l].n);
+    }
+    o_m1_end = cur;
+  };
+  layout(0);
+  uint32_t lean = 0;
+  if (tl_forward_lean_enabled()) {
+    Run P = R;
+    P.probing = true;
+    P.g0 = P.ar.take(4 * cur);
+    P.network();
+    if (P.rc != TL_OK) return P.rc;
+    for (int l = 0; l < nl; ++l)
+      if (R.lv[l].ct >= 0 && !(P.need_table >> l & 1)) lean |= 1u << l;
+    if (lean) layout(lean);
+  }
+  a->lean_levels = (int32_t)lean;
   R.g0 = R.ar.take(4 * cur);
 
   {
diff --git a/treelearn_amd/csrc/tl_voxel.hip b/treelearn_amd/csrc/tl_voxel.hip
--- a/treelearn_amd/csrc/tl_voxel.hip
+++ b/treelearn_amd/csrc/tl_voxel.hip
@@ -509,9 +509,11 @@
           if (bit < 63) { if (word & (2ull << bit)) r2 = (int)(base + __popcll(word & ((below << 1) | 1ull))); }
           else if (z + 1 < d.Z) r2 = tl_rank_at(bm, pf, wc, z + 1);
         }
-        nbr[(int64_t)(tap0 + 0) * M + i] = r0;
-        nbr[(int64_t)(tap0 + 1) * M + i] = r1;
-        nbr[(int64_t)(tap0 + 2) * M + i] = r2;
+        if (nbr) {
+          nbr[(int64_t)(tap0 + 0) * M + i] = r0;
+          nbr[(int64_t)(tap0 + 1) * M + i] = r1;
+          nbr[(int64_t)(tap0 + 2) * M + i] = r2;
+        }
         if (compact) {
           compact[(int64_t)(tap0 / 3) * M + i] = r0 >= 0 ? r0 : (r1 >= 0 ? r1 : r2);
           cmask |= ((r0 >= 0 ? 1u : 0u) | (r1 >= 0 ? 2u : 0u) | (r2 >= 0 ? 4u : 0u)) << tap0;
@@ -866,8 +868,8 @@
   if (!lv || num_levels < 1 || num_levels > kPyrMaxLevels) return TL_ERR_ARG;
   for (int l = 0; l < num_levels; ++l) {
     if (!lv[l].bitmap || !lv[l].prefix || lv[l].n <= 0) return TL_ERR_ARG;
-    if ((!lv[l].coords || !lv[l].nbr) && !lv[l].o2n) return TL_ERR_ARG;
-    if (lv[l].nbr && !lv[l].coords) return TL_ERR_ARG;
+    if ((!lv[l].coords || (!lv[l].nbr && !lv[l].compact)) && !lv[l].o2n) return TL_ERR_ARG;
+    if ((lv[l].nbr || lv[l].compact) && !lv[l].coords) return TL_ERR_ARG;
     if (l > 0 && !lv[l].coords) return TL_ERR_ARG;
     if (l + 1 < num_levels && (!lv[l].child || (!lv[l].inv && !lv[l].inv_packed))) return TL_ERR_ARG;
     if (lv[l].inv_packed && lv[l].n >= (1ll << 28)) return TL_ERR_ARG;
@@ -889,7 +891,7 @@
   for (int l = 0; l < small; ++l) {
     const TlDims d = tl_dims(lv[l].dims);
     if (lv[l].coords) k_expand_coords<<<tl_grid(tl_nwords(d), kBlock), kBlock, 0, s>>>(lv[l].bitmap, lv[l].prefix, d, lv[l].coords);
-    if (lv[l].nbr) k_rulebook_subm<<<tl_grid(lv[l].n, kBlock), kBlock, 0, s>>>(lv[l].coords, lv[l].n, lv[l].bitmap, lv[l].prefix, d, lv[l].nbr, lv[l].compact);
+    if (lv[l].nbr || lv[l].compact) k_rulebook_subm<<<tl_grid(lv[l].n, kBlock), kBlock, 0, s>>>(lv[l].coords, lv[l].n, lv[l].bitmap, lv[l].prefix, d, lv[l].nbr, lv[l].compact);
   }
   LevelPack p;
   p.nl = num_levels - small;
diff --git a/treelearn_amd/model/executor.py b/treelearn_amd/model/executor.py
--- a/treelearn_amd/model/executor.py
+++ b/treelearn_amd/model/executor.py
@@ -258,5 +258,6 @@
         if rc == _hip.TL_ERR_EXTENT:
             raise ValueError("voxelize: tile extent exceeds spatial_shape, batch id out of range or voxel coordinate outside [0, 65536)")
         _hip.check(rc, "tl_forward")
-        self.last = dict(level_n=list(a.level_n[:self.desc.num_levels]), blocked=bool(a.blocked_used), launches=a.launches, arena_bytes=a.needed_bytes)
+        self.last = dict(level_n=list(a.level_n[:self.desc.num_levels]), blocked=bool(a.blocked_used), launches=a.launches, arena_bytes=a.needed_bytes,
+                         lean_levels=int(a.lean_levels))
         return bb, logits, offsets
```

Result: no change. 258.9 Mpoints/s, median of 6 (+0.5%).
